# antgroup/ant-ray

Hardware: NVIDIA H100
Metric: resnet50_ddp_train_images_per_sec (higher is better)
Workload: dtype bf16

## Files before the change

ant-ray_b200/_native.py:

```python
import ctypes
import os
from ctypes import (POINTER, Structure, byref, c_char_p, c_float, c_int, c_int32, c_size_t, c_uint8,
                    c_uint32, c_uint64, c_void_p)

_LIB_NAME = "libb200coll.so"
_lib = None


class B200CollError(RuntimeError):

    def __init__(self, status, message):
        super().__init__(message)
        self.status = status

    def __reduce__(self):
        return (B200CollError, (self.status, self.args[0] if self.args else ""))


OK, EINVAL, ECUDA, ESTATE, EUNSUPPORTED, ETIMEOUT, EABORTED, EMISMATCH, ENOMEM = 0, -1, -2, -3, -4, -5, -6, -7, -8
INT8, UINT8, INT32, UINT32, INT64, UINT64, FLOAT16, FLOAT32, FLOAT64, BFLOAT16 = range(10)
SUM, PROD, MAX, MIN, AVG = range(5)
ALGO_AUTO, ALGO_ONESHOT, ALGO_TWOSHOT, ALGO_NVLS, ALGO_NVLS_PIPE, ALGO_LL, ALGO_NVLS_LANES, ALGO_NVLS_STREAMS = range(8)
SHARE_VMM_FD, SHARE_LEGACY_IPC = 0, 1
ACT_RELU6, ACT_SILU, ACT_HARDSWISH = 1, 2, 3
MAX_RANKS = 8


class Config(Structure):
    _fields_ = [("struct_size", c_uint32), ("share_mode", c_int32), ("staging_bytes", c_uint64),
                ("symmetric_bytes", c_uint64), ("p2p_slot_bytes", c_uint64), ("p2p_slots", c_uint32),
                ("max_blocks", c_uint32), ("oneshot_max_bytes", c_uint64), ("nvls_min_bytes", c_uint64),
                ("nvls_pipe_min_bytes", c_uint64), ("timeout_ms", c_uint64), ("granule_bytes", c_uint64),
                ("ll_max_bytes", c_uint64), ("bcast_rounds_min_bytes", c_uint64), ("nvls_blocks", c_uint32),
                ("nvls_lanes", c_uint32), ("lane_granule_bytes", c_uint64), ("nvls_lanes_min_bytes", c_uint64),
                ("nvls_unroll", c_uint32), ("rounds_order", c_uint32), ("nvls_streams_min_bytes", c_uint64),
                ("nvls_streams_piece_bytes", c_uint64)]


class Props(Structure):
    _fields_ = [("device", c_int32), ("sm_count", c_int32), ("cc_major", c_int32), ("cc_minor", c_int32),
                ("vmm_supported", c_int32), ("posix_fd_supported", c_int32), ("multicast_supported", c_int32),
                ("reserved", c_int32), ("total_mem", c_uint64)]


class Export(Structure):
    _fields_ = [("share_mode", c_int32), ("fd", c_int32), ("arena_bytes", c_uint64), ("layout_hash", c_uint64),
                ("pid", c_int32), ("device_uuid_lo", c_int32), ("ipc", c_uint8 * 64)]


SYMBOLS = {
    "b200c_version": (c_int, []),
    "b200c_last_error": (c_char_p, []),
    "b200c_status_string": (c_char_p, [c_int]),
    "b200c_dtype_size": (c_size_t, [c_int]),
    "b200c_device_props": (c_int, [c_int, POINTER(Props)]),
    "b200c_default_config": (None, [POINTER(Config)]),
    "b200c_comm_create": (c_int, [c_int, c_int, c_int, POINTER(Config), POINTER(c_void_p)]),
    "b200c_comm_export": (c_int, [c_void_p, POINTER(Export)]),
    "b200c_comm_import": (c_int, [c_void_p, c_int, POINTER(Export)]),
    "b200c_comm_mc_create": (c_int, [c_void_p, POINTER(c_int)]),
    "b200c_comm_mc_import": (c_int, [c_void_p, c_int]),
    "b200c_comm_mc_add_device": (c_int, [c_void_p]),
    "b200c_comm_mc_bind": (c_int, [c_void_p]),
    "b200c_comm_mc_disable": (c_int, [c_void_p]),
    "b200c_comm_ready": (c_int, [c_void_p]),
    "b200c_comm_abort": (c_int, [c_void_p]),
    "b200c_comm_destroy": (c_int, [c_void_p]),
    "b200c_comm_check": (c_int, [c_void_p]),
    "b200c_comm_rank": (c_int, [c_void_p]),
    "b200c_comm_world": (c_int, [c_void_p]),
    "b200c_comm_has_multicast": (c_int, [c_void_p]),
    "b200c_comm_seq": (c_uint64, [c_void_p]),
    "b200c_comm_symmetric_base": (c_void_p, [c_void_p]),
    "b200c_comm_symmetric_bytes": (c_uint64, [c_void_p]),
    "b200c_pool_bind": (c_int, [c_void_p]),
    "b200c_pool_malloc": (c_void_p, [c_size_t, c_int, c_void_p]),
    "b200c_pool_free": (None, [c_void_p, c_size_t, c_int, c_void_p]),
    "b200c_allreduce": (c_int, [c_void_p, c_void_p, c_void_p, c_size_t, c_int, c_int, c_int, c_void_p]),
    "b200c_allreduce_scaled": (c_int, [c_void_p, c_void_p, c_void_p, c_size_t, c_int, c_int, c_float, c_int, c_void_p]),
    "b200c_reduce": (c_int, [c_void_p, c_void_p, c_void_p, c_size_t, c_int, c_int, c_int, c_void_p]),
    "b200c_broadcast": (c_int, [c_void_p, c_void_p, c_size_t, c_int, c_int, c_void_p]),
    "b200c_allgather": (c_int, [c_void_p, c_void_p, POINTER(c_void_p), c_size_t, c_int, c_void_p]),
    "b200c_reducescatter": (c_int, [c_void_p, POINTER(c_void_p), c_void_p, c_size_t, c_int, c_int, c_void_p]),
    "b200c_reducescatter_scaled": (c_int, [c_void_p, POINTER(c_void_p), c_void_p, c_size_t, c_int, c_int, c_float, c_void_p]),
    "b200c_send": (c_int, [c_void_p, c_void_p, c_size_t, c_int, c_void_p]),
    "b200c_recv": (c_int, [c_void_p, c_void_p, c_size_t, c_int, c_void_p]),
    "b200c_send_multi": (c_int, [c_void_p, c_void_p, c_size_t, POINTER(c_int), c_int, c_void_p]),
    "b200c_recv_multi": (c_int, [c_void_p, c_void_p, c_size_t, c_int, c_void_p]),
    "b200c_barrier": (c_int, [c_void_p, c_void_p]),
    "b200c_debug_fill_flags": (c_int, [c_void_p, c_uint32]),
    "b200c_bn_scratch_bytes": (c_size_t, [c_int]),
    "b200c_bn_forward": (c_int, [c_void_p] * 10 + [c_int, c_int, c_float, c_float, c_void_p, c_void_p]),
    "b200c_bn_forward_mask": (c_int, [c_void_p] * 11 + [c_int, c_int, c_float, c_float, c_void_p, c_void_p]),
    "b200c_bn_backward": (c_int, [c_void_p] * 10 + [c_int, c_int, c_void_p, c_void_p]),
    "b200c_bn_backward_mask": (c_int, [c_void_p] * 11 + [c_int, c_int, c_void_p, c_void_p]),
    "b200c_bn_dual_scratch_bytes": (c_size_t, [c_int]),
    "b200c_bn_forward_dual": (c_int, [c_void_p] * 11 + [c_float, c_float] + [c_void_p] * 7 + [c_float, c_float, c_int, c_int, c_void_p, c_void_p]),
    "b200c_bn_backward_dual": (c_int, [c_void_p] * 18 + [c_int, c_int, c_void_p, c_void_p]),
    "b200c_bn_forward_pool": (c_int, [c_void_p] * 10 + [c_int] * 4 + [c_float, c_float, c_void_p, c_void_p]),
    "b200c_bn_backward_pool": (c_int, [c_void_p] * 10 + [c_int] * 4 + [c_void_p, c_void_p]),
    "b200c_bn_infer": (c_int, [c_void_p] * 7 + [c_int, c_float, c_int, c_int, c_void_p]),
    "b200c_bn_infer_dual": (c_int, [c_void_p] * 7 + [c_float] + [c_void_p] * 4 + [c_float, c_int, c_int, c_int, c_void_p]),
    "b200c_bn_infer_pool": (c_int, [c_void_p] * 6 + [c_int, c_float] + [c_int] * 4 + [c_void_p]),
    "b200c_bn_forward_act": (c_int, [c_void_p] * 9 + [c_int, c_int, c_int, c_float, c_float, c_void_p, c_void_p]),
    "b200c_bn_backward_act": (c_int, [c_void_p] * 10 + [c_int, c_int, c_int, c_void_p, c_void_p]),
    "b200c_bn_infer_act": (c_int, [c_void_p] * 6 + [c_int, c_float, c_int, c_int, c_int, c_void_p]),
    "b200c_bn_forward_res": (c_int, [c_void_p] * 3 + [c_int] + [c_void_p] * 8 + [c_int, c_int, c_float, c_float, c_void_p, c_void_p]),
    "b200c_bn_backward_res": (c_int, [c_void_p] * 2 + [c_int] + [c_void_p] * 8 + [c_int, c_int, c_void_p, c_void_p]),
    "b200c_bn_infer_res": (c_int, [c_void_p] * 7 + [c_int, c_float, c_int, c_int, c_void_p]),
    "b200c_bn_forward_cat": (c_int, [POINTER(c_void_p), POINTER(c_int), c_int] + [c_void_p] * 9 + [c_int, c_int, c_float, c_float, c_void_p,
                                                                                              c_void_p]),
    "b200c_bn_backward_cat": (c_int, [c_void_p] * 2 + [POINTER(c_void_p), POINTER(c_int), c_int] + [c_void_p] * 6 + [c_int, c_int, c_void_p,
                                                                                                                  c_void_p]),
    "b200c_bn_infer_cat": (c_int, [POINTER(c_void_p), POINTER(c_int), c_int] + [c_void_p] * 5 + [c_int, c_float, c_int, c_int, c_void_p]),
    "b200c_bn_forward_slice": (c_int, [c_void_p, c_void_p, c_int] + [c_void_p] * 8 + [c_int, c_int, c_float, c_float, c_void_p, c_void_p]),
    "b200c_bn_backward_slice": (c_int, [c_void_p, c_int] + [c_void_p] * 8 + [c_int, c_int, c_void_p, c_void_p]),
    "b200c_bn_infer_slice": (c_int, [c_void_p, c_void_p, c_int] + [c_void_p] * 4 + [c_int, c_float, c_int, c_int, c_void_p]),
    "b200c_bn_shuffle_mask_bytes": (c_size_t, [c_int, c_int]),
    "b200c_bn_forward_shuffle": (c_int, [c_void_p, c_int] + [c_void_p] * 9 + [c_float, c_float] + [c_void_p] * 9
                                 + [c_float, c_float, c_void_p, c_int, c_int, c_int, c_void_p, c_void_p]),
    "b200c_bn_backward_shuffle": (c_int, [c_void_p] * 17 + [c_int, c_int, c_void_p, c_void_p]),
    "b200c_bn_infer_shuffle": (c_int, [c_void_p, c_int] + [c_void_p] * 5 + [c_float] + [c_void_p] * 5
                               + [c_float, c_void_p, c_int, c_int, c_int, c_int, c_void_p]),
    "b200c_se_scratch_bytes": (c_size_t, [c_int, c_int, c_int]),
    "b200c_se_pool": (c_int, [c_void_p] * 2 + [c_int] * 3 + [c_void_p, c_size_t, c_void_p]),
    "b200c_se_scale": (c_int, [c_void_p] * 3 + [c_int] * 3 + [c_void_p]),
    "b200c_se_backward_reduce": (c_int, [c_void_p] * 3 + [c_int] * 3 + [c_void_p, c_size_t, c_void_p]),
    "b200c_se_backward_elemt": (c_int, [c_void_p] * 4 + [c_int] * 3 + [c_void_p]),
    "b200c_bn_sync_scratch_bytes": (c_size_t, [c_int, c_int]),
    "b200c_bn_sync_forward": (c_int, [c_void_p] * 5 + [c_int] + [c_void_p] * 8 + [c_int, c_int, c_float, c_float, c_void_p, c_void_p]),
    "b200c_bn_sync_backward": (c_int, [c_void_p] * 5 + [c_int] + [c_void_p] * 9 + [c_int, c_int, c_void_p, c_void_p]),
    "b200c_launch_count": (c_uint64, []),
}


def library_path():
    override = os.environ.get("B200COLL_LIBRARY")
    if override:
        return override
    return os.path.join(os.path.dirname(os.path.abspath(__file__)), _LIB_NAME)


def load():
    global _lib
    if _lib is not None:
        return _lib
    path = library_path()
    if not os.path.exists(path):
        raise ImportError(
            f"{path} not found: build it with `python -c 'import __graft_entry__ as g; g.build()'` "
            "(nvcc, sm_90a).  ant_ray_b200 has no CPU or NCCL fallback.")
    lib = ctypes.CDLL(path, mode=ctypes.RTLD_LOCAL)
    for name, (restype, argtypes) in SYMBOLS.items():
        fn = getattr(lib, name)
        fn.restype = restype
        fn.argtypes = argtypes
    if lib.b200c_version() < 200:
        raise ImportError("libb200coll.so is older than this Python package")
    _lib = lib
    return lib


def last_error():
    msg = load().b200c_last_error()
    return msg.decode(errors="replace") if msg else ""


def check(status):
    if status != OK:
        raise B200CollError(status, f"b200coll: {last_error()} (status {status})")


def default_config():
    cfg = Config()
    load().b200c_default_config(byref(cfg))
    return cfg


def device_props(device):
    p = Props()
    check(load().b200c_device_props(device, byref(p)))
    return p


def launch_count():
    return int(load().b200c_launch_count())
```

ant-ray_b200/csrc/b200coll.cu:

```cuda
#include <cuda.h>
#include <cuda_runtime.h>
#include <stdarg.h>
#include <stdio.h>
#include <stdlib.h>
#include <string.h>
#include <unistd.h>

#include <atomic>
#include <initializer_list>
#include <mutex>

#include "byte_kernels.cuh"
#include "launch_typed.cuh"
#include "norm_launch.h"
#include "se_launch.h"

using namespace b200c;

static thread_local char g_err[512] = "";
static int fail(int code, const char* fmt, ...) {
  va_list ap;
  va_start(ap, fmt);
  vsnprintf(g_err, sizeof g_err, fmt, ap);
  va_end(ap);
// ... 934 lines not shown
      c->tma_ctas_per_sm = nb;
    }
    size_t cap = (size_t)c->sm_count * c->tma_ctas_per_sm;
    int tgrid = (int)(ntiles < cap ? ntiles : cap);
    with_scaled_types(dtype, wire, [&](auto ti, auto tw) {
      k_local_scale_tma<typename decltype(ti)::type, typename decltype(tw)::type><<<tgrid, kTmaThreads, kTmaSmemBytes, s>>>(a);
    });
    int rc = launch_check(c, "local_scale_tma");
    if (rc) return rc;
    if (tma_elems == count) return B200C_OK;
    a.in = static_cast<const char*>(send) + tma_elems * esz;
    a.out = static_cast<char*>(recv) + tma_elems * esz;
    a.n = count - tma_elems;
  }
  int grid = local_scale_grid<float, bf16_t>(c, a.n * esz);
  if (dtype == B200C_FLOAT64) k_local_scale<double, double><<<grid, kThreads, 0, s>>>(a);
  else if (!with_scaled_types(dtype, wire, [&](auto ti, auto tw) {
             k_local_scale<typename decltype(ti)::type, typename decltype(tw)::type><<<grid, kThreads, 0, s>>>(a);
           }))
    return copy_if_distinct(send, recv, count * esz, s);
  return launch_check(c, "local_scale");
}

static int choose_algo(b200c_comm* c, int algo, size_t total_bytes, size_t bytes_left, bool ll_ok, bool nvls_ok, bool in_sym,
                       bool* pipe, bool* lanes) {
  const int W = c->world;
  int al = algo;
  if (al == B200C_ALGO_NVLS_PIPE) { al = B200C_ALGO_NVLS; *pipe = true; }
  if (al == B200C_ALGO_NVLS_LANES) { al = B200C_ALGO_NVLS; *lanes = true; }
  if (al == B200C_ALGO_AUTO) {
    if (ll_ok && total_bytes <= c->cfg.ll_max_bytes) al = B200C_ALGO_LL;
    else if (bytes_left <= c->cfg.oneshot_max_bytes) al = B200C_ALGO_ONESHOT;
    else if (nvls_ok && W > 2 && bytes_left >= c->cfg.nvls_min_bytes && (W >= 6 || in_sym)) al = B200C_ALGO_NVLS;
    else al = B200C_ALGO_TWOSHOT;
  }
  return al;
}

static void plan_ll(b200c_comm* c, CollArgs& a, size_t left, size_t esz, size_t vec, int& grid) {
  size_t n = left;
  a.chunk = round_up(n, vec);
  a.tile = vec;
  a.ll_seq = c->ll_seq + 1;
  size_t nvec = (n * esz + 15) / 16;
  size_t nb = (nvec + kLLThreads - 1) / kLLThreads;
  grid = (int)(nb < 1 ? 1 : (nb > c->cfg.max_blocks ? c->cfg.max_blocks : nb));
  a.n = n;
}
static void plan_oneshot(b200c_comm* c, CollArgs& a, size_t left, size_t wsz, size_t vec, int& grid) {
  const int W = c->world;
  size_t cap = c->cfg.staging_bytes / W / wsz / vec * vec;
  size_t n = left < cap ? left : cap;
  a.chunk = round_up(n, vec);
  plan_tiles(n, wsz, vec, c->cfg.max_blocks, kMinTileBytes, c->cfg.granule_bytes, &a.tile, &grid);
  a.n = n;
}
static void plan_twoshot(b200c_comm* c, CollArgs& a, size_t left, size_t wsz, size_t vec, int& grid) {
  const int W = c->world;
  size_t cap_chunk = c->cfg.staging_bytes / W / wsz / vec * vec;
  size_t cap = cap_chunk * W;
  size_t n = left < cap ? left : cap;
  a.chunk = round_up((n + W - 1) / W, vec);
  plan_tiles(a.chunk, wsz, vec, c->cfg.max_blocks, kMinTileBytes, c->cfg.granule_bytes, &a.tile, &grid);
  a.n = n;
}
static int plan_nvls(b200c_comm* c, CollArgs& a, size_t left, size_t wsz, size_t vec, bool sym, int algo, bool& pipe, bool& lanes,
                     int& grid, uint32_t& rounds) {
  const int W = c->world;
  const uint32_t nvls_sym_cap = c->cfg.nvls_blocks && c->cfg.nvls_blocks < c->cfg.max_blocks ? c->cfg.nvls_blocks : c->cfg.max_blocks;
  size_t cap = sym ? ((size_t)256 << 20) / wsz : c->cfg.staging_bytes / wsz / vec * vec;
  size_t n = left < cap ? left : cap;
  a.chunk = round_up((n + W - 1) / W, vec);
  a.symmetric = sym ? 1 : 0;
  a.sym_off = sym ? (size_t)((const char*)a.in - c->arena[c->rank]) : 0;
  if (!sym && algo == B200C_ALGO_AUTO && c->cfg.nvls_lanes_min_bytes && left * wsz >= c->cfg.nvls_lanes_min_bytes) lanes = true;
  if (!sym && !lanes && algo == B200C_ALGO_AUTO && c->cfg.nvls_pipe_min_bytes && n * wsz >= c->cfg.nvls_pipe_min_bytes) pipe = true;
  if (sym) pipe = lanes = false;
  if (lanes) {
    n = left;
    a.chunk = round_up((n + W - 1) / W, vec);
    uint32_t L = c->cfg.nvls_lanes;
    uint32_t Kc = c->cfg.max_blocks / L - 1;
    if (Kc > 7) Kc = 7;
    if (Kc < 1) Kc = 1;
    size_t tb = c->cfg.lane_granule_bytes, chunk_bytes = a.chunk * wsz;
    size_t want = chunk_bytes / ((size_t)L * 4) / 8192 * 8192;
    if (want < 8192) want = 8192;
    if (tb > want) tb = want;
    size_t ring = (size_t)L * kLaneSlots * W * tb;
    while (ring > c->cfg.staging_bytes && tb > 8192) { tb -= 8192; ring = (size_t)L * kLaneSlots * W * tb; }
    while (ring > c->cfg.staging_bytes && L > 1) { L--; ring = (size_t)L * kLaneSlots * W * tb; }
    if (ring > c->cfg.staging_bytes) return fail(B200C_EINVAL, "staging_bytes too small for the lane kernel's ring (%zu bytes)", ring);
    a.tile = tb / wsz;
    a.lane_copy = (int)Kc;
    size_t ngran = (a.chunk + a.tile - 1) / a.tile;
    uint32_t used = (uint32_t)(ngran < L ? ngran : L);
    grid = (int)(used * (1 + Kc));
    rounds = (uint32_t)((ngran + used - 1) / used);
    a.pipe_base = c->pipe_base;
  } else if (pipe) {
    plan_rounds(a.chunk, wsz, vec, c->cfg.max_blocks, c->cfg.granule_bytes, &a.tile, &grid, &rounds);
    a.pipe_base = c->pipe_base;
  } else {
    plan_tiles(a.chunk, wsz, vec, sym ? nvls_sym_cap : c->cfg.max_blocks, kMinTileBytes, c->cfg.granule_bytes, &a.tile, &grid);
  }
  a.n = n;
  return B200C_OK;
}

static int allreduce_impl(b200c_comm* c, const void* send, void* recv, size_t count, int dtype, int wire, int op, float scale,
                          int has_scale, int algo, cudaStream_t s) {
  int rc = check_ready(c);
  if (rc) return rc;
  size_t esz = b200c_dtype_size(dtype), wsz = b200c_dtype_size(wire);
  if (!esz || !wsz) return fail(B200C_EINVAL, "bad dtype %d / wire %d", dtype, wire);
  if (op < 0 || op >= B200C_NUM_OPS) return fail(B200C_EINVAL, "bad reduce op %d", op);
  if (count && (!send || !recv)) return fail(B200C_EINVAL, "null buffer");
  if (wire != dtype) {
    if (!(dtype == B200C_FLOAT32 && (wire == B200C_BFLOAT16 || wire == B200C_FLOAT16))) return fail(B200C_EUNSUPPORTED, "wire dtype %d for buffer dtype %d", wire, dtype);
    if (op != B200C_SUM && op != B200C_AVG) return fail(B200C_EUNSUPPORTED, "compressed wire supports SUM/AVG only");
  }
  if (algo < B200C_ALGO_AUTO || algo > B200C_ALGO_NVLS_STREAMS) return fail(B200C_EINVAL, "bad algo %d", algo);
  if (op == B200C_AVG) { has_scale = 1; scale = 1.f / (float)c->world; }
  if (count == 0) return B200C_OK;
  DeviceGuard g(c->device);
  const int W = c->world;
  const size_t vec = 16 / wsz;
  if (W == 1) return allreduce_local(c, send, recv, count, dtype, wire, scale, has_scale, s);

  const bool nvls_ok = c->mc_arena && (op == B200C_SUM || op == B200C_AVG) &&
                       (wire == B200C_FLOAT32 || wire == B200C_BFLOAT16 || wire == B200C_FLOAT16);
  if ((algo == B200C_ALGO_NVLS || algo == B200C_ALGO_NVLS_PIPE || algo == B200C_ALGO_NVLS_LANES || algo == B200C_ALGO_NVLS_STREAMS) && !nvls_ok) return fail(B200C_EUNSUPPORTED, "NVLS needs a bound multicast object, SUM/AVG and f32/bf16/f16");
  const bool ll_ok = wire == dtype && c->ll_words && count * esz <= c->ll_words * 4;
  if (algo == B200C_ALGO_LL && !ll_ok) return fail(B200C_EUNSUPPORTED, "LL needs wire == dtype and at most %zu bytes (ll_max_bytes)", c->ll_words * 4);
  const char* in = static_cast<const char*>(send);
  char* out = static_cast<char*>(recv);
  bool in_sym = false;
  if (wire == dtype && send == recv && c->sym_bytes && (((uintptr_t)send) & 15) == 0 && (count * esz) % 16 == 0) {
    const char* base = c->arena[c->rank] + c->off_sym;
    in_sym = in >= base && in + count * esz <= base + c->sym_bytes;
  }
  if (!in_sym && (algo == B200C_ALGO_NVLS_STREAMS ||
                  (algo == B200C_ALGO_AUTO && nvls_ok && W >= 6 && c->cfg.nvls_streams_min_bytes && count * wsz >= c->cfg.nvls_streams_min_bytes)))
    return allreduce_streams(c, send, recv, count, dtype, wire, op, scale, has_scale, s);
  return run_pieces(c, count, count, "allreduce", [&](CollArgs& a, size_t done, uint32_t& rounds) -> int {
    const size_t left = count - done;
    bool pipe = false, lanes = false;
    const int al = choose_algo(c, algo, count * esz, left * wsz, ll_ok, nvls_ok, in_sym, &pipe, &lanes);
    a.in = in + done * esz; a.out = out + done * esz;
    a.has_scale = has_scale; a.scale = scale;
    const bool sym = al == B200C_ALGO_NVLS && in_sym;
    int grid = 0;
    if (al == B200C_ALGO_LL) plan_ll(c, a, left, esz, vec, grid);
    else if (al == B200C_ALGO_ONESHOT) plan_oneshot(c, a, left, wsz, vec, grid);
    else if (al == B200C_ALGO_TWOSHOT) plan_twoshot(c, a, left, wsz, vec, grid);
    else {
      int rc = plan_nvls(c, a, left, wsz, vec, sym, algo, pipe, lanes, grid, rounds);
      if (rc) return rc;
    }
    a.sig = make_sig(OPC_ALLREDUCE, dtype * 16 + wire, op, a.n, sym ? (int)((a.sym_off >> 4) & 0x3fffffff) : -1, al * 8 + (sym ? 1 : 0) + (pipe ? 2 : 0) + (lanes ? 4 : 0));
    if (al == B200C_ALGO_NVLS) launch_nvls(dtype, wire, a, grid, s, pipe, lanes);
    else if (wire != dtype) {
      if (wire == B200C_BFLOAT16) launch_mixed<float, bf16_t>(al, a, grid, s);
      else launch_mixed<float, f16_t>(al, a, grid, s);
    } else {
      int kind = al == B200C_ALGO_LL ? KIND_LL : (al == B200C_ALGO_ONESHOT ? KIND_ONESHOT : KIND_TWOSHOT);
      return launch_same_type(dtype, kind, op, a, grid, s);
    }
    return B200C_OK;
  });
}

extern "C" int b200c_allreduce(b200c_comm_t* c, const void* send, void* recv, size_t count, int dtype, int op, int algo,
                               b200c_stream_t stream) {
  return allreduce_impl(c, send, recv, count, dtype, dtype, op, 1.f, 0, algo, (cudaStream_t)stream);
}

extern "C" int b200c_allreduce_scaled(b200c_comm_t* c, const void* send, void* recv, size_t count, int dtype, int wire_dtype,
                                      float scale, int algo, b200c_stream_t stream) {
  if (dtype != B200C_FLOAT32 && dtype != B200C_BFLOAT16 && dtype != B200C_FLOAT16)
    return fail(B200C_EUNSUPPORTED, "scaled allreduce supports f32/bf16/f16 buffers, got %d", dtype);
  return allreduce_impl(c, send, recv, count, dtype, wire_dtype, B200C_SUM, scale, 1, algo, (cudaStream_t)stream);
}

extern "C" int b200c_reduce(b200c_comm_t* c, const void* send, void* recv, size_t count, int dtype, int op, int root,
                            b200c_stream_t stream) {
  int rc = check_ready(c);
  if (rc) return rc;
  size_t esz = b200c_dtype_size(dtype);
  if (!esz) return fail(B200C_EINVAL, "bad dtype %d", dtype);
  if (op < 0 || op >= B200C_NUM_OPS) return fail(B200C_EINVAL, "bad reduce op %d", op);
  if (root < 0 || root >= c->world) return fail(B200C_EINVAL, "bad root %d", root);
  if (count == 0) return B200C_OK;
  if (!send || (c->rank == root && !recv)) return fail(B200C_EINVAL, "null buffer");
  cudaStream_t s = (cudaStream_t)stream;
  DeviceGuard g(c->device);
  if (c->world == 1) return copy_if_distinct(send, recv, count * esz, s);
  const size_t vec = 16 / esz;
  size_t cap = c->cfg.staging_bytes / c->world / esz / vec * vec;
  return run_pieces(c, count, cap, "reduce", [&](CollArgs& a, size_t done, uint32_t&) {
    a.in = static_cast<const char*>(send) + done * esz;
    a.out = recv ? static_cast<char*>(recv) + done * esz : nullptr;
    a.chunk = round_up(a.n, vec); a.root = root;
    if (op == B200C_AVG) { a.has_scale = 1; a.scale = 1.f / c->world; }
    int grid;
    plan_tiles(a.n, esz, vec, c->cfg.max_blocks, kMinTileBytes, c->cfg.granule_bytes, &a.tile, &grid);
    a.sig = make_sig(OPC_REDUCE, dtype, op, a.n, root, 0);
    return launch_same_type(dtype, KIND_REDUCE, op, a, grid, s);
  });
}

extern "C" int b200c_reducescatter(b200c_comm_t* c, const void* const* send_ptrs, void* recv, size_t count, int dtype, int op,
                                   b200c_stream_t stream) {
  int rc = check_ready(c);
  if (rc) return rc;
  size_t esz = b200c_dtype_size(dtype);
  if (!esz) return fail(B200C_EINVAL, "bad dtype %d", dtype);
  if (op < 0 || op >= B200C_NUM_OPS) return fail(B200C_EINVAL, "bad reduce op %d", op);
  if (count == 0) return B200C_OK;
  if (!send_ptrs || !recv) return fail(B200C_EINVAL, "null buffer");
  for (int j = 0; j < c->world; j++) if (!send_ptrs[j]) return fail(B200C_EINVAL, "send_ptrs[%d] is null", j);
  cudaStream_t s = (cudaStream_t)stream;
  DeviceGuard g(c->device);
  if (c->world == 1) return copy_if_distinct(send_ptrs[0], recv, count * esz, s);
  const size_t vec = 16 / esz;
  size_t cap = c->cfg.staging_bytes / c->world / esz / vec * vec;
  return run_pieces(c, count, cap, "reducescatter", [&](CollArgs& a, size_t done, uint32_t&) {
    for (int j = 0; j < c->world; j++) a.in_ptrs[j] = static_cast<const char*>(send_ptrs[j]) + done * esz;
    a.out = static_cast<char*>(recv) + done * esz;
    a.chunk = round_up(a.n, vec);
    if (op == B200C_AVG) { a.has_scale = 1; a.scale = 1.f / c->world; }
    int grid;
    plan_tiles(a.n, esz, vec, c->cfg.max_blocks, kMinTileBytes, c->cfg.granule_bytes, &a.tile, &grid);
    a.sig = make_sig(OPC_REDUCESCATTER, dtype, op, a.n, -1, 0);
    return launch_same_type(dtype, KIND_REDUCESCATTER, op, a, grid, s);
  });
}

extern "C" int b200c_reducescatter_scaled(b200c_comm_t* c, const void* const* send_ptrs, void* recv, size_t count, int dtype,
                                          int wire_dtype, float scale, b200c_stream_t stream) {
  int rc = check_ready(c);
  if (rc) return rc;
  if (dtype != B200C_FLOAT32 && dtype != B200C_BFLOAT16 && dtype != B200C_FLOAT16)
    return fail(B200C_EUNSUPPORTED, "scaled reducescatter supports f32/bf16/f16 buffers, got %d", dtype);
  const size_t esz = b200c_dtype_size(dtype), wsz = b200c_dtype_size(wire_dtype);
  if (!wsz) return fail(B200C_EINVAL, "bad wire dtype %d", wire_dtype);
  if (wire_dtype != dtype && !(dtype == B200C_FLOAT32 && (wire_dtype == B200C_BFLOAT16 || wire_dtype == B200C_FLOAT16)))
    return fail(B200C_EUNSUPPORTED, "wire dtype %d for buffer dtype %d", wire_dtype, dtype);
  if (count == 0) return B200C_OK;
  if (!send_ptrs || !recv) return fail(B200C_EINVAL, "null buffer");
  for (int j = 0; j < c->world; j++) if (!send_ptrs[j]) return fail(B200C_EINVAL, "send_ptrs[%d] is null", j);
  cudaStream_t s = (cudaStream_t)stream;
  if (c->world == 1) return allreduce_impl(c, send_ptrs[0], recv, count, dtype, wire_dtype, B200C_SUM, scale, 1, B200C_ALGO_AUTO, s);
  DeviceGuard g(c->device);
  const size_t vec = 16 / wsz;
  size_t cap = c->cfg.staging_bytes / c->world / wsz / vec * vec;
  return run_pieces(c, count, cap, "reducescatter_scaled", [&](CollArgs& a, size_t done, uint32_t&) {
    for (int j = 0; j < c->world; j++) a.in_ptrs[j] = static_cast<const char*>(send_ptrs[j]) + done * esz;
    a.out = static_cast<char*>(recv) + done * esz;
    a.chunk = round_up(a.n, vec);
    a.has_scale = 1; a.scale = scale;
    int grid;
    plan_tiles(a.n, wsz, vec, c->cfg.max_blocks, kMinTileBytes, c->cfg.granule_bytes, &a.tile, &grid);
    a.sig = make_sig(OPC_REDUCESCATTER, dtype, B200C_SUM, a.n, -1, 16 + wire_dtype);
    launch_rs_scaled(dtype, wire_dtype, a, grid, s);
    return B200C_OK;
  });
}

extern "C" int b200c_allgather(b200c_comm_t* c, const void* send, void* const* recv_ptrs, size_t count, int dtype,
                               b200c_stream_t stream) {
  int rc = check_ready(c);
  if (rc) return rc;
  size_t esz = b200c_dtype_size(dtype);
  if (!esz) return fail(B200C_EINVAL, "bad dtype %d", dtype);
  if (count == 0) return B200C_OK;
  if (!send || !recv_ptrs) return fail(B200C_EINVAL, "null buffer");
  for (int j = 0; j < c->world; j++) if (!recv_ptrs[j]) return fail(B200C_EINVAL, "recv_ptrs[%d] is null", j);
  cudaStream_t s = (cudaStream_t)stream;
  DeviceGuard g(c->device);
  size_t bytes = count * esz;
  if (c->world == 1) return copy_if_distinct(send, recv_ptrs[0], bytes, s);
  size_t cap = c->cfg.staging_bytes / c->world / 16 * 16;
  return run_pieces(c, bytes, cap, "allgather", [&](CollArgs& a, size_t done, uint32_t&) {
    a.in = static_cast<const char*>(send) + done;
    for (int j = 0; j < c->world; j++) a.out_ptrs[j] = static_cast<char*>(recv_ptrs[j]) + done;
    a.chunk = round_up(a.n, 16);
    int grid;
    plan_tiles(a.n, 1, 16, c->cfg.max_blocks, kMinTileBytes, c->cfg.granule_bytes, &a.tile, &grid);
    a.sig = make_sig(OPC_ALLGATHER, dtype, 0, a.n, -1, 0);
    k_allgather<<<grid, kThreads, 0, s>>>(a);
    return B200C_OK;
  });
}

extern "C" size_t b200c_bn_scratch_bytes(int channels) {
  return channels < 1 || channels > bn::kMaxChannels ? 0 : bn::scratch_bytes(channels);
}

extern "C" size_t b200c_bn_sync_scratch_bytes(int channels, int world) {
  return channels < 1 || channels > bn::kMaxChannels || world < 1 || world > kMaxRanks ? 0 : bn::sync_scratch_bytes(channels, world);
}

static const char* bn_site(bool sync) { return sync ? "sync batch norm" : "batch norm"; }

static int check_bn(const char* site, int min_m, int m, int c, const void* scratch, int relu, const void* mask, const void* residual,
                    const void* dy2) {
  if (m < min_m || c < 1 || c > bn::kMaxChannels || (int64_t)m * c > INT32_MAX)
    return fail(B200C_EINVAL, "%s: bad shape m=%d c=%d", site, m, c);
  if (!scratch) return fail(B200C_EINVAL, "%s: null scratch", site);
  if (!relu && (mask || residual || dy2)) return fail(B200C_EINVAL, "%s: a site without ReLU takes no mask, identity or dy2", site);
  if (mask && c % 8) return fail(B200C_EINVAL, "%s mask: channels=%d is not a multiple of 8", site, c);
  return B200C_OK;
}

static int bn_forward(b200c_comm_t* comm, bool sync, const void* x, const void* identity, void* y, void* mask, int relu,
                      const float* weight, const float* bias, float* running_mean, float* running_var, int64_t* num_batches_tracked,
                      float* save_mean, float* save_invstd, float* norm_fct, int m, int channels, float momentum, float eps,
                      void* scratch, b200c_stream_t stream) {
  int rc = check_bn(bn_site(sync), sync ? 0 : 1, m, channels, scratch, relu, mask, identity, nullptr);
  if (rc) return rc;
  if ((m && (!x || !y)) || !weight || !bias || !running_mean || !running_var || !save_mean || !save_invstd || (sync && !norm_fct))
    return fail(B200C_EINVAL, "%s forward: null buffer", bn_site(sync));
  const bn::FwdArgs a{x, identity, y, mask, relu != 0, weight, bias, running_mean, running_var,
                      reinterpret_cast<long long*>(num_batches_tracked), save_mean, save_invstd, m, channels, momentum, eps, scratch};
  cudaStream_t s = (cudaStream_t)stream;
  if (!sync) {
    RT(bn::forward(a, s));
    g_launches.fetch_add(2);
    return B200C_OK;
  }
  rc = check_ready(comm);
  if (rc) return rc;
  DeviceGuard g(comm->device);
  const int rows = m != 0;
  RT(bn::sync_stats(a, s));
  g_launches.fetch_add(rows);
  const bn::SyncRows r = bn::sync_rows(scratch, channels);
  void* gathered[kMaxRanks];
  for (int j = 0; j < comm->world; j++) gathered[j] = r.gathered + j * r.row_floats;
  rc = b200c_allgather(comm, r.local, gathered, (size_t)2 * channels + 1, B200C_FLOAT32, stream);
  if (rc) return rc;
  RT(bn::sync_apply(a, comm->world, norm_fct, s));
  g_launches.fetch_add(1 + rows);
  return B200C_OK;
}

static int bn_backward(b200c_comm_t* comm, bool sync, const void* dy, const void* dy2, const void* y, const void* mask, int relu,
                       const void* x, void* dy_masked, void* dx, const float* weight, const float* save_mean, const float* save_invstd,
                       const float* norm_fct, float* grad_weight, float* grad_bias, int m, int channels, void* scratch,
                       b200c_stream_t stream) {
  int rc = check_bn(bn_site(sync), sync ? 0 : 1, m, channels, scratch, relu, mask, dy_masked, dy2);
  if (rc) return rc;
  if ((m && (!dy || !x || !dx || (relu && !y && !mask))) || !weight || !save_mean || !save_invstd || (sync && !norm_fct) ||
      !grad_weight || !grad_bias)
    return fail(B200C_EINVAL, "%s backward: null buffer", bn_site(sync));
  const bn::BwdArgs a{dy, dy2, y, mask, x, dy_masked, dx, relu != 0, weight, save_mean, save_invstd, norm_fct, grad_weight, grad_bias,
                      m, channels, scratch};
  cudaStream_t s = (cudaStream_t)stream;
  if (!sync) {
    RT(bn::backward(a, s));
    g_launches.fetch_add(2);
    return B200C_OK;
  }
  rc = check_ready(comm);
  if (rc) return rc;
  DeviceGuard g(comm->device);
  const int rows = m != 0;
  RT(bn::sync_bwd_reduce(a, s));
  g_launches.fetch_add(rows);
  float* sums = bn::sync_rows(scratch, channels).sums;
  rc = b200c_allreduce(comm, sums, sums, (size_t)2 * channels, B200C_FLOAT32, B200C_SUM, B200C_ALGO_AUTO, stream);
  if (rc) return rc;
  RT(bn::sync_bwd_elemt(a, s));
  g_launches.fetch_add(rows);
  return B200C_OK;
}

extern "C" int b200c_bn_forward(const void* x, const void* identity, void* y, const float* weight, const float* bias,
                                float* running_mean, float* running_var, int64_t* num_batches_tracked, float* save_mean,
                                float* save_invstd, int m, int channels, float momentum, float eps, void* scratch,
                                b200c_stream_t stream) {
  return bn_forward(nullptr, false, x, identity, y, nullptr, 1, weight, bias, running_mean, running_var, num_batches_tracked, save_mean,
                    save_invstd, nullptr, m, channels, momentum, eps, scratch, stream);
}

extern "C" int b200c_bn_forward_mask(const void* x, const void* identity, void* y, uint8_t* mask, const float* weight,
                                     const float* bias, float* running_mean, float* running_var, int64_t* num_batches_tracked,
                                     float* save_mean, float* save_invstd, int m, int channels, float momentum, float eps,
                                     void* scratch, b200c_stream_t stream) {
  if (!mask) return fail(B200C_EINVAL, "batch norm mask: null mask");
  return bn_forward(nullptr, false, x, identity, y, mask, 1, weight, bias, running_mean, running_var, num_batches_tracked, save_mean,
                    save_invstd, nullptr, m, channels, momentum, eps, scratch, stream);
}

extern "C" int b200c_bn_sync_forward(b200c_comm_t* comm, const void* x, const void* identity, void* y, uint8_t* mask, int relu,
                                     const float* weight, const float* bias, float* running_mean, float* running_var,
                                     int64_t* num_batches_tracked, float* save_mean, float* save_invstd, float* norm_fct, int m,
                                     int channels, float momentum, float eps, void* scratch, b200c_stream_t stream) {
  return bn_forward(comm, true, x, identity, y, mask, relu, weight, bias, running_mean, running_var, num_batches_tracked, save_mean,
                    save_invstd, norm_fct, m, channels, momentum, eps, scratch, stream);
}

extern "C" int b200c_bn_backward(const void* dy, const void* y, const void* x, void* dy_masked, void* dx, const float* weight,
                                 const float* save_mean, const float* save_invstd, float* grad_weight, float* grad_bias, int m,
                                 int channels, void* scratch, b200c_stream_t stream) {
  return bn_backward(nullptr, false, dy, nullptr, y, nullptr, 1, x, dy_masked, dx, weight, save_mean, save_invstd, nullptr, grad_weight,
                     grad_bias, m, channels, scratch, stream);
}

extern "C" int b200c_bn_backward_mask(const void* dy, const void* dy2, const uint8_t* mask, const void* x, void* dy_masked,
                                      void* dx, const float* weight, const float* save_mean, const float* save_invstd,
                                      float* grad_weight, float* grad_bias, int m, int channels, void* scratch,
                                      b200c_stream_t stream) {
  if (!mask) return fail(B200C_EINVAL, "batch norm mask: null mask");
  return bn_backward(nullptr, false, dy, dy2, nullptr, mask, 1, x, dy_masked, dx, weight, save_mean, save_invstd, nullptr, grad_weight,
                     grad_bias, m, channels, scratch, stream);
}

extern "C" int b200c_bn_sync_backward(b200c_comm_t* comm, const void* dy, const void* dy2, const void* y, const uint8_t* mask, int relu,
                                      const void* x, void* dy_masked, void* dx, const float* weight, const float* save_mean,
                                      const float* save_invstd, const float* norm_fct, float* grad_weight, float* grad_bias, int m,
                                      int channels, void* scratch, b200c_stream_t stream) {
  return bn_backward(comm, true, dy, dy2, y, mask, relu, x, dy_masked, dx, weight, save_mean, save_invstd, norm_fct, grad_weight,
                     grad_bias, m, channels, scratch, stream);
}

extern "C" size_t b200c_bn_dual_scratch_bytes(int channels) {
  return channels < 1 || channels > bn::kMaxChannels / 2 ? 0 : bn::dual_scratch_bytes(channels);
}

static int check_dual(int channels) {
  if (channels > bn::kMaxChannels / 2) return fail(B200C_EINVAL, "batch norm dual: channels=%d above %d", channels, bn::kMaxChannels / 2);
  return B200C_OK;
}

extern "C" int b200c_bn_forward_dual(const void* x, const void* x_ds, void* y, uint8_t* mask, const float* weight, const float* bias,
                                     float* running_mean, float* running_var, int64_t* num_batches_tracked, float* save_mean,
                                     float* save_invstd, float momentum, float eps, const float* weight_ds, const float* bias_ds,
                                     float* running_mean_ds, float* running_var_ds, int64_t* num_batches_tracked_ds,
                                     float* save_mean_ds, float* save_invstd_ds, float momentum_ds, float eps_ds, int m, int channels,
                                     void* scratch, b200c_stream_t stream) {
  int rc = check_bn("batch norm dual", 1, m, channels, scratch, 1, mask, x_ds, nullptr);
  if (!rc) rc = check_dual(channels);
  if (rc) return rc;
  if (!x || !x_ds || !y || !weight || !bias || !running_mean || !running_var || !save_mean || !save_invstd || !weight_ds ||
      !bias_ds || !running_mean_ds || !running_var_ds || !save_mean_ds || !save_invstd_ds)
    return fail(B200C_EINVAL, "batch norm dual forward: null buffer");
  const bn::FwdArgs a{x, nullptr, y, mask, true, weight, bias, running_mean, running_var,
                      reinterpret_cast<long long*>(num_batches_tracked), save_mean, save_invstd, m, channels, momentum, eps, scratch};
  const bn::FwdArgs b{x_ds, nullptr, nullptr, nullptr, false, weight_ds, bias_ds, running_mean_ds, running_var_ds,
                      reinterpret_cast<long long*>(num_batches_tracked_ds), save_mean_ds, save_invstd_ds, m, channels, momentum_ds,
                      eps_ds, scratch};
  RT(bn::forward_dual(a, b, (cudaStream_t)stream));
  g_launches.fetch_add(2);
  return B200C_OK;
}

extern "C" int b200c_bn_backward_dual(const void* dy, const void* dy2, const void* y, const uint8_t* mask, const void* x,
                                      const void* x_ds, void* dx, void* dx_ds, const float* weight, const float* save_mean,
                                      const float* save_invstd, float* grad_weight, float* grad_bias, const float* weight_ds,
                                      const float* save_mean_ds, const float* save_invstd_ds, float* grad_weight_ds,
                                      float* grad_bias_ds, int m, int channels, void* scratch, b200c_stream_t stream) {
  int rc = check_bn("batch norm dual", 1, m, channels, scratch, 1, mask, nullptr, dy2);
  if (!rc) rc = check_dual(channels);
  if (rc) return rc;
  if (!dy || (!y && !mask) || !x || !x_ds || !dx || !dx_ds || !weight || !save_mean || !save_invstd || !grad_weight || !grad_bias ||
      !weight_ds || !save_mean_ds || !save_invstd_ds || !grad_weight_ds || !grad_bias_ds)
    return fail(B200C_EINVAL, "batch norm dual backward: null buffer");
  const bn::BwdArgs a{dy, dy2, mask ? nullptr : y, mask, x, nullptr, dx, true, weight, save_mean, save_invstd, nullptr, grad_weight,
                      grad_bias, m, channels, scratch};
  const bn::BwdArgs b{nullptr, nullptr, nullptr, nullptr, x_ds, nullptr, dx_ds, false, weight_ds, save_mean_ds, save_invstd_ds, nullptr,
                      grad_weight_ds, grad_bias_ds, m, channels, scratch};
  RT(bn::backward_dual(a, b, (cudaStream_t)stream));
  g_launches.fetch_add(2);
  return B200C_OK;
}

static int check_pool(const char* dir, int n, int h, int w, int channels, int* m) {
  if (n < 1 || h < 1 || w < 1 || (int64_t)n * h * w > INT32_MAX)
    return fail(B200C_EINVAL, "batch norm pool %s: bad shape n=%d h=%d w=%d c=%d", dir, n, h, w, channels);
  *m = n * h * w;
  return B200C_OK;
}

extern "C" int b200c_bn_forward_pool(const void* x, void* y, uint8_t* argmax, const float* weight, const float* bias,
                                     float* running_mean, float* running_var, int64_t* num_batches_tracked, float* save_mean,
                                     float* save_invstd, int n, int h, int w, int channels, float momentum, float eps, void* scratch,
                                     b200c_stream_t stream) {
  int m = 0;
  int rc = check_pool("forward", n, h, w, channels, &m);
  if (!rc) rc = check_bn("batch norm pool", 1, m, channels, scratch, 1, nullptr, nullptr, nullptr);
  if (rc) return rc;
  if (!x || !y || !argmax || !weight || !bias || !running_mean || !running_var || !save_mean || !save_invstd)
    return fail(B200C_EINVAL, "batch norm pool forward: null buffer");
  bn::FwdArgs a{x, nullptr, y, nullptr, true, weight, bias, running_mean, running_var,
                reinterpret_cast<long long*>(num_batches_tracked), save_mean, save_invstd, m, channels, momentum, eps, scratch};
  a.argmax = argmax;
  a.pool_h = h;
  a.pool_w = w;
  RT(bn::forward(a, (cudaStream_t)stream));
  g_launches.fetch_add(2);
  return B200C_OK;
}

extern "C" int b200c_bn_backward_pool(const void* dy, const uint8_t* argmax, const void* x, void* g, void* dx, const float* weight,
                                      const float* save_mean, const float* save_invstd, float* grad_weight, float* grad_bias, int n,
                                      int h, int w, int channels, void* scratch, b200c_stream_t stream) {
  int m = 0;
  int rc = check_pool("backward", n, h, w, channels, &m);
  if (!rc) rc = check_bn("batch norm pool", 1, m, channels, scratch, 1, nullptr, nullptr, nullptr);
  if (rc) return rc;
  if (!dy || !argmax || !x || !g || !dx || !weight || !save_mean || !save_invstd || !grad_weight || !grad_bias)
    return fail(B200C_EINVAL, "batch norm pool backward: null buffer");
  bn::BwdArgs a{dy, nullptr, nullptr, nullptr, x, g, dx, true, weight, save_mean, save_invstd, nullptr, grad_weight, grad_bias,
                m, channels, scratch};
  a.argmax = argmax;
  a.pool_h = h;
  a.pool_w = w;
  RT(bn::backward(a, (cudaStream_t)stream));
  g_launches.fetch_add(2);
  return B200C_OK;
}

static int check_infer(const char* site, int param_bf16, int m, int c) {
  if (m < 1 || c < 1 || (int64_t)m * c > INT32_MAX) return fail(B200C_EINVAL, "%s: bad shape m=%d c=%d", site, m, c);
  if (param_bf16 != 0 && param_bf16 != 1) return fail(B200C_EINVAL, "%s: param_bf16=%d is neither 0 nor 1", site, param_bf16);
  return B200C_OK;
}

static int run_infer(const bn::InferArgs& a, b200c_stream_t stream) {
  RT(bn::infer(a, (cudaStream_t)stream));
  g_launches.fetch_add(1);
  return B200C_OK;
}

extern "C" int b200c_bn_infer(const void* x, const void* identity, void* y, const void* weight, const void* bias,
                              const void* running_mean, const void* running_var, int param_bf16, float eps, int m, int channels,
                              b200c_stream_t stream) {
  int rc = check_infer("batch norm infer", param_bf16, m, channels);
  if (rc) return rc;
  if (!x || !y || !weight || !bias || !running_mean || !running_var) return fail(B200C_EINVAL, "batch norm infer: null buffer");
  return run_infer({x, identity, y, {weight, bias, running_mean, running_var, eps}, {}, false, param_bf16 != 0, m, channels, 0, 0},
                   stream);
}

extern "C" int b200c_bn_infer_dual(const void* x, const void* x_ds, void* y, const void* weight, const void* bias,
                                   const void* running_mean, const void* running_var, float eps, const void* weight_ds,
                                   const void* bias_ds, const void* running_mean_ds, const void* running_var_ds, float eps_ds,
                                   int param_bf16, int m, int channels, b200c_stream_t stream) {
  int rc = check_infer("batch norm infer dual", param_bf16, m, channels);
  if (rc) return rc;
  if (!x || !x_ds || !y || !weight || !bias || !running_mean || !running_var || !weight_ds || !bias_ds || !running_mean_ds ||
      !running_var_ds)
    return fail(B200C_EINVAL, "batch norm infer dual: null buffer");
  return run_infer({x, x_ds, y, {weight, bias, running_mean, running_var, eps}, {weight_ds, bias_ds, running_mean_ds, running_var_ds, eps_ds},
                    true, param_bf16 != 0, m, channels, 0, 0},
                   stream);
}

extern "C" int b200c_bn_infer_pool(const void* x, void* y, const void* weight, const void* bias, const void* running_mean,
                                   const void* running_var, int param_bf16, float eps, int n, int h, int w, int channels,
                                   b200c_stream_t stream) {
  int m = 0;
  int rc = check_pool("infer", n, h, w, channels, &m);
  if (!rc) rc = check_infer("batch norm infer pool", param_bf16, m, channels);
  if (rc) return rc;
  if (!x || !y || !weight || !bias || !running_mean || !running_var) return fail(B200C_EINVAL, "batch norm infer pool: null buffer");
  return run_infer({x, nullptr, y, {weight, bias, running_mean, running_var, eps}, {}, false, param_bf16 != 0, m, channels, h, w}, stream);
}

static int check_act(const char* site, int act, int c) {
  if (!bn::act_ok(act)) return fail(B200C_EINVAL, "%s: unknown act=%d", site, act);
  if (c > bn::kMaxChannels) return fail(B200C_EINVAL, "%s: channels=%d above %d", site, c, bn::kMaxChannels);
  return B200C_OK;
}

extern "C" int b200c_bn_forward_act(const void* x, void* y, const float* weight, const float* bias, float* running_mean,
                                    float* running_var, int64_t* num_batches_tracked, float* save_mean, float* save_invstd, int act,
                                    int m, int channels, float momentum, float eps, void* scratch, b200c_stream_t stream) {
  int rc = check_bn("batch norm act", 1, m, channels, scratch, 1, nullptr, nullptr, nullptr);
  if (!rc) rc = check_act("batch norm act", act, channels);
  if (rc) return rc;
  if (!x || !y || !weight || !bias || !running_mean || !running_var || !save_mean || !save_invstd)
    return fail(B200C_EINVAL, "batch norm act forward: null buffer");
  const bn::FwdArgs a{x, nullptr, y, nullptr, false, weight, bias, running_mean, running_var,
                      reinterpret_cast<long long*>(num_batches_tracked), save_mean, save_invstd, m, channels, momentum, eps, scratch};
  RT(bn::forward_act(a, act, (cudaStream_t)stream));
  g_launches.fetch_add(2);
  return B200C_OK;
}

extern "C" int b200c_bn_backward_act(const void* dy, const void* x, void* g, void* dx, const float* weight, const float* bias,
                                     const float* save_mean, const float* save_invstd, float* grad_weight, float* grad_bias, int act,
                                     int m, int channels, void* scratch, b200c_stream_t stream) {
  int rc = check_bn("batch norm act", 1, m, channels, scratch, 1, nullptr, nullptr, nullptr);
  if (!rc) rc = check_act("batch norm act", act, channels);
  if (rc) return rc;
  if (!dy || !x || !g || !dx || !weight || !bias || !save_mean || !save_invstd || !grad_weight || !grad_bias)
    return fail(B200C_EINVAL, "batch norm act backward: null buffer");
  const bn::BwdArgs a{dy, nullptr, nullptr, nullptr, x, g, dx, false, weight, save_mean, save_invstd, nullptr, grad_weight, grad_bias,
                      m, channels, scratch};
  RT(bn::backward_act(a, bias, act, (cudaStream_t)stream));
  g_launches.fetch_add(2);
  return B200C_OK;
}
// ... 461 lines not shown
```

ant-ray_b200/csrc/inst_norm.cu:

```cuda
#include <algorithm>
#include <initializer_list>
#include <type_traits>

#include "norm_act.cuh"
#include "norm_cat.cuh"
#include "norm_infer.cuh"
#include "norm_kernels.cuh"
#include "norm_launch.h"
#include "norm_res.cuh"
#include "norm_shuffle.cuh"
#include "norm_slice.cuh"

namespace b200c {
namespace bn {

static int ceil_div(int a, int b) { return (a + b - 1) / b; }

static int last_pow2(unsigned n) {
  n |= (n >> 1);
  n |= (n >> 2);
  n |= (n >> 4);
  n |= (n >> 8);
  n |= (n >> 16);
  return std::max<int>(1, n - (n >> 1));
}

static void reduce_config(int reduction, int stride, dim3* block, dim3* grid) {
  int block_x = std::min(last_pow2(stride), kTileW);
  int block_y = std::min(last_pow2(ceil_div(reduction, kElemsPerThread)), kMaxBlock / block_x);
  if (block_x * block_y != kMaxBlock) block_x = std::min(last_pow2(stride), kMaxBlock / block_y);
  int grid_y = std::min(ceil_div(reduction, block_y * kElemsPerThread), kMaxHBlock);
  *block = dim3(block_x, block_y, 1);
  *grid = dim3(ceil_div(stride, block_x), grid_y < 8 ? 1 : grid_y, 1);
}

static_assert(kEwVec % kStatsVec == 0, "vec_ok covers the statistics kernel's vector width");
static bool vec_ok(int stride, const void* const* ptrs, int n) {
  if (stride % kEwVec) return false;
  for (int i = 0; i < n; i++)
    if (reinterpret_cast<uintptr_t>(ptrs[i]) % 16) return false;
  return true;
}

constexpr size_t kBlockSmem = 48 * 1024;
constexpr size_t kStatsStaticSmem = 3 * kMaxBlock * 4 + 16;
constexpr size_t kBwdStaticSmem = 2 * kMaxBlock * 4 + 16;

static size_t stats_ring_bytes(dim3 block) {
  return (size_t)kStatsStages * kParallelLoads * block.x * block.y * sizeof(BVec<kStatsVec>);
}
static_assert(kStatsStaticSmem + (size_t)kStatsStages * kParallelLoads * (kMaxBlock / kStatsVec) * sizeof(BVec<kStatsVec>) <= kBlockSmem,
              "the statistics ring fits every block");

static_assert(kBwdStaticSmem + (size_t)kBwdStagesWide * 5 * kParallelLoads * (kMaxBlock / kBwdVec) * sizeof(BVec<kBwdVec>) <= kBlockSmem &&
                  kBwdStaticSmem + (size_t)kBwdStages * 2 * kParallelLoads * (kMaxBlock / kBwdVec) * sizeof(BVec<kBwdVec>) <= kBlockSmem,
              "the backward ring fits every block: 2 stages of up to 5 operands, 3 of 2");
struct BwdReduceLaunch {
  dim3 block, grid;
  int vec;
  size_t smem;
};
static BwdReduceLaunch bwd_reduce_launch(int m, int c, GradSrc src, bool dy2, bool dual, const void* const* ptrs, int n) {
  BwdReduceLaunch l;
  reduce_config(m, c, &l.block, &l.grid);
  l.vec = 1;
  l.smem = 0;
  if (src == kGradPool || !vec_ok(c, ptrs, n)) return l;
  const int ops = bwd_ring_operands(src == kGradY, dy2, dual);
  const size_t ring = (size_t)bwd_ring_stages(ops) * ops * kParallelLoads * (l.block.x / kBwdVec) * l.block.y * sizeof(BVec<kBwdVec>);
  l.block.x /= kBwdVec;
  l.vec = kBwdVec;
  l.smem = ring;
  return l;
}

static void ew_config(int reduction, int stride, int vec, dim3* block, dim3* grid) {
  const int groups = stride / vec;
  const int bx = std::min(groups, kEwThreads);
  const int by = kEwThreads / bx;
  const int gx = ceil_div(groups, bx);
  const int gy = std::max(1, std::min(ceil_div(reduction, by), 4096 / gx));
  *block = dim3(bx, by, 1);
  *grid = dim3(gx, gy, 1);
}

constexpr int kSemaphores = kMaxChannels / kTileW;
constexpr size_t kSemaphoreBytes = (size_t)kSemaphores * 4;

size_t scratch_bytes(int stride) {
  return kSemaphoreBytes + (size_t)3 * stride * kMaxHBlock * 4 + (size_t)2 * stride * 4;
}

struct Scratch {
  int* semaphores;
  float* staging;
  float* sums;
};
static Scratch carve(void* scratch, int stride) {
  char* p = static_cast<char*>(scratch);
  Scratch s;
  s.semaphores = reinterpret_cast<int*>(p);
  s.staging = reinterpret_cast<float*>(p + kSemaphoreBytes);
  s.sums = s.staging + (size_t)3 * stride * kMaxHBlock;
  return s;
}

template <int... Cs, typename F>
static auto with_const(int key, F&& f) {
  std::common_type_t<decltype(f(std::integral_constant<int, Cs>{}))...> kernel = nullptr;
  ((key == Cs ? void(kernel = f(std::integral_constant<int, Cs>{})) : void()), ...);
  return kernel;
}

using StatsKernel = void (*)(const bf16*, StatsOut, volatile float*, int*, int, int);
using SyncStatsKernel = void (*)(const bf16*, float*, float, volatile float*, int*, int, int);
using StatsDualKernel = void (*)(const bf16*, const bf16*, StatsOut, StatsOut, volatile float*, volatile float*, int*, int, int);
using TransformKernel = void (*)(const bf16*, const bf16*, bf16*, uint8_t*, const float*, const float*, const float*, const float*,
                                 const float*, const float*, const float*, const float*, int, int);
using PoolFwdKernel = void (*)(const bf16*, bf16*, uint8_t*, const float*, const float*, const float*, const float*, PoolDims, int, int);
using BwdReduceKernel = void (*)(const bf16*, const bf16*, const bf16*, const bf16*, const uint8_t*, bf16*, const float*, const float*,
                                 float*, float*, float*, float*, volatile float*, int*, PoolDims, const bf16*, const float*, const float*,
                                 float*, float*, float*, int, int, int);
using BwdElemtKernel = void (*)(const bf16*, const bf16*, const bf16*, const uint8_t*, const bf16*, bf16*, const float*, const float*,
                                const float*, const float*, const float*, const float*, float, const bf16*, bf16*, const float*,
                                const float*, const float*, const float*, int, int);

static StatsKernel stats_kernel(int vec) {
  return with_const<1, kStatsVec>(vec, [](auto v) -> StatsKernel { return k_bn_stats<decltype(v)::value>; });
}
static StatsDualKernel stats_dual_kernel(int vec) {
  return with_const<1, kStatsVec>(vec, [](auto v) -> StatsDualKernel { return k_bn_stats_dual<decltype(v)::value>; });
}
static SyncStatsKernel sync_stats_kernel(int vec) {
  return with_const<1, kStatsVec>(vec, [](auto v) -> SyncStatsKernel { return k_bn_sync_stats<decltype(v)::value>; });
}
static TransformKernel transform_kernel(int vec, int tail) {
  return with_const<1, kEwVec>(vec, [&](auto v) {
    return with_const<kTailNone, kTailRelu, kTailAddRelu, kTailBnAddRelu>(
        tail, [](auto t) -> TransformKernel { return k_bn_transform<decltype(v)::value, (Tail) decltype(t)::value>; });
  });
}
static PoolFwdKernel pool_fwd_kernel(int vec) {
  return with_const<1, kEwVec>(vec, [](auto v) -> PoolFwdKernel { return k_bn_pool_fwd<decltype(v)::value>; });
}
static BwdReduceKernel bwd_reduce_kernel(int src, bool dual) {
  if (dual)
    return with_const<kGradY, kGradBits>(src, [](auto g) -> BwdReduceKernel { return k_bn_bwd_reduce<(GradSrc) decltype(g)::value, true>; });
  return with_const<kGradY, kGradBits, kGradDy, kGradPool>(
      src, [](auto g) -> BwdReduceKernel { return k_bn_bwd_reduce<(GradSrc) decltype(g)::value, false>; });
}
static BwdElemtKernel bwd_elemt_kernel(int vec, int src, bool fct_ptr, bool dual) {
  return with_const<1, kEwVec>(vec, [&](auto v) {
    if (dual)
      return with_const<kGradY, kGradBits>(src, [](auto g) -> BwdElemtKernel {
        return k_bn_bwd_elemt<decltype(v)::value, (GradSrc) decltype(g)::value, false, true>;
      });
    return with_const<kGradMasked, kGradY, kGradBits, kGradDy>(src, [&](auto g) {
      auto kernel = [](auto p) -> BwdElemtKernel {
        return k_bn_bwd_elemt<decltype(v)::value, (GradSrc) decltype(g)::value, decltype(p)::value != 0, false>;
      };
      if constexpr (decltype(g)::value == kGradDy) return with_const<true>(fct_ptr, kernel);
      else return with_const<false, true>(fct_ptr, kernel);
    });
  });
}

template <typename P>
using InferTransformKernel = void (*)(const bf16*, const bf16*, bf16*, const P*, const P*, const P*, const P*, float, const P*, const P*,
                                      const P*, const P*, float, int, int);
template <typename P>
using InferPoolKernel = void (*)(const bf16*, bf16*, const P*, const P*, const P*, const P*, float, PoolDims, int, int);

template <typename P>
static InferTransformKernel<P> infer_transform_kernel(int vec, int tail) {
  return with_const<1, kEwVec>(vec, [&](auto v) {
    return with_const<kTailRelu, kTailAddRelu, kTailBnAddRelu>(tail, [](auto t) -> InferTransformKernel<P> {
      return bn_infer::k_infer_transform<decltype(v)::value, (Tail) decltype(t)::value, P>;
    });
  });
}
template <typename P>
static InferPoolKernel<P> infer_pool_kernel(int vec) {
  return with_const<1, kEwVec>(vec, [](auto v) -> InferPoolKernel<P> { return bn_infer::k_infer_pool<decltype(v)::value, P>; });
}

using bn_act::Act;
using ActTransformKernel = void (*)(const bf16*, bf16*, const float*, const float*, const float*, const float*, int, int);
using ActBwdReduceKernel = void (*)(const bf16*, const bf16*, const float*, const float*, const float*, const float*, float*, float*,
                                    float*, float*, volatile float*, int*, bf16*, int, int);
template <typename P>
using ActInferKernel = void (*)(const bf16*, bf16*, const P*, const P*, const P*, const P*, float, int, int);

template <typename F>
static auto with_act(int act, F&& f) {
  return with_const<bn_act::kActRelu6, bn_act::kActSilu, bn_act::kActHardswish>(act, f);
}
bool act_ok(int act) { return act == bn_act::kActRelu6 || act == bn_act::kActSilu || act == bn_act::kActHardswish; }

static ActTransformKernel act_transform_kernel(int vec, int act) {
  return with_const<1, kEwVec>(vec, [&](auto v) {
    return with_act(act, [](auto a) -> ActTransformKernel { return bn_act::k_act_transform<decltype(v)::value, (Act) decltype(a)::value>; });
  });
}
static ActBwdReduceKernel act_bwd_reduce_kernel(int act) {
  return with_act(act, [](auto a) -> ActBwdReduceKernel { return bn_act::k_act_bwd_reduce<(Act) decltype(a)::value>; });
}
template <typename P>
static ActInferKernel<P> act_infer_kernel(int vec, int act) {
  return with_const<1, kEwVec>(vec, [&](auto v) {
    return with_act(act, [](auto a) -> ActInferKernel<P> { return bn_act::k_act_infer<decltype(v)::value, (Act) decltype(a)::value, P>; });
  });
}

using bn_res::Res;
using ResTransformKernel = void (*)(const bf16*, const bf16*, const bf16*, bf16*, const float*, const float*, const float*, const float*,
                                    int, int, int);
using ResBwdReduceKernel = void (*)(const bf16*, const bf16*, const bf16*, const float*, const float*, float*, float*, float*, float*,
                                    volatile float*, int*, bf16*, int, int, int);
template <typename P>
using ResInferKernel = void (*)(const bf16*, const bf16*, bf16*, const P*, const P*, const P*, const P*, float, int, int);

static ResTransformKernel res_transform_kernel(int vec, bool drop) {
  return with_const<1, kEwVec>(vec, [&](auto v) -> ResTransformKernel {
    return drop ? bn_res::k_res_transform<decltype(v)::value, bn_res::kResDropAdd> : bn_res::k_res_transform<decltype(v)::value, bn_res::kResAdd>;
  });
}
static ResBwdReduceKernel res_bwd_reduce_kernel() { return bn_res::k_res_bwd_reduce; }
template <typename P>
static ResInferKernel<P> res_infer_kernel(int vec, bool add) {
  return with_const<1, kEwVec>(vec, [&](auto v) -> ResInferKernel<P> {
    return add ? bn_res::k_res_infer<decltype(v)::value, bn_res::kResAdd, P> : bn_res::k_res_infer<decltype(v)::value, bn_res::kResPlain, P>;
  });
}

cudaError_t load_kernels() {
  cudaFuncAttributes attr;
  cudaError_t e = cudaSuccess;
  auto load = [&](auto kernel) { if (kernel && e == cudaSuccess) e = cudaFuncGetAttributes(&attr, kernel); };
  load(&k_bn_sync_merge);
  load(res_bwd_reduce_kernel());
  load(&bn_cat::k_cat_stats);
  load(&bn_cat::k_cat_transform);
  load(&bn_cat::k_cat_bwd_reduce);
  load(&bn_cat::k_cat_bwd_elemt);
  load(&bn_cat::k_cat_infer<float>);
  load(&bn_cat::k_cat_infer<bf16>);
  load(&bn_slice::k_slice_transform);
  load(&bn_slice::k_slice_bwd_reduce);
  load(&bn_slice::k_slice_bwd_elemt);
  load(&bn_slice::k_slice_infer<float>);
  load(&bn_slice::k_slice_infer<bf16>);
  load(&bn_shuffle::k_shuffle_transform<false>);
  load(&bn_shuffle::k_shuffle_transform<true>);
  load(&bn_shuffle::k_shuffle_bwd_reduce<false>);
  load(&bn_shuffle::k_shuffle_bwd_reduce<true>);
  load(&bn_shuffle::k_shuffle_bwd_elemt<false>);
  load(&bn_shuffle::k_shuffle_bwd_elemt<true>);
  load(&bn_shuffle::k_shuffle_infer<false, float>);
  load(&bn_shuffle::k_shuffle_infer<true, float>);
  load(&bn_shuffle::k_shuffle_infer<false, bf16>);
  load(&bn_shuffle::k_shuffle_infer<true, bf16>);
  for (int src = 0; src < kGradSrcs; src++) {
    load(bwd_reduce_kernel(src, false));
    load(bwd_reduce_kernel(src, true));
  }
  for (int vec : {1, kStatsVec, kEwVec}) {
    load(stats_kernel(vec));
    load(stats_dual_kernel(vec));
    load(sync_stats_kernel(vec));
    load(pool_fwd_kernel(vec));
    for (int tail = 0; tail < kTails; tail++) load(transform_kernel(vec, tail));
    for (int src = 0; src < kGradSrcs; src++)
      for (bool fct_ptr : {false, true})
        for (bool dual : {false, true}) load(bwd_elemt_kernel(vec, src, fct_ptr, dual));
    load(infer_pool_kernel<float>(vec));
    load(infer_pool_kernel<bf16>(vec));
    for (int tail = 0; tail < kTails; tail++) {
      load(infer_transform_kernel<float>(vec, tail));
      load(infer_transform_kernel<bf16>(vec, tail));
    }
    for (int act : {bn_act::kActRelu6, bn_act::kActSilu, bn_act::kActHardswish}) {
      if (vec == 1) load(act_bwd_reduce_kernel(act));
      load(act_transform_kernel(vec, act));
      load(act_infer_kernel<float>(vec, act));
      load(act_infer_kernel<bf16>(vec, act));
    }
    for (bool b : {false, true}) {
      load(res_transform_kernel(vec, b));
      load(res_infer_kernel<float>(vec, b));
      load(res_infer_kernel<bf16>(vec, b));
    }
  }
  return e;
}

constexpr cudaError_t kNoKernel = cudaErrorInvalidDeviceFunction;

static cudaError_t launch_stats(const FwdArgs& a, float* sync_row, cudaStream_t st) {
  Scratch s = carve(a.scratch, a.c);
  dim3 block, grid;
  reduce_config(a.m, a.c, &block, &grid);
  const int vec = vec_ok(a.c, &a.x, 1) ? kStatsVec : 1;
  block.x /= vec;
  const size_t smem = vec == kStatsVec ? stats_ring_bytes(block) : 0;
  const bf16* x = static_cast<const bf16*>(a.x);
  if (sync_row) {
    const SyncStatsKernel k = sync_stats_kernel(vec);
    if (!k) return kNoKernel;
    k<<<grid, block, smem, st>>>(x, sync_row, a.eps, s.staging, s.semaphores, a.m, a.c);
  } else {
    const StatsKernel k = stats_kernel(vec);
    if (!k) return kNoKernel;
    StatsOut o{a.save_mean, a.save_invstd, a.running_mean, a.running_var, a.num_batches_tracked, a.momentum,
               (float)((double)a.m / (double)(a.m - 1)), a.eps};
    k<<<grid, block, smem, st>>>(x, o, s.staging, s.semaphores, a.m, a.c);
  }
  return cudaGetLastError();
}

static cudaError_t launch_transform(const FwdArgs& a, cudaStream_t st) {
  const void* ptrs[3] = {a.x, a.y, a.identity ? a.identity : a.x};
  const int vec = vec_ok(a.c, ptrs, 3) ? kEwVec : 1;
  dim3 block, grid;
  ew_config(a.m, a.c, vec, &block, &grid);
  const TransformKernel k = transform_kernel(vec, !a.relu ? kTailNone : a.identity ? kTailAddRelu : kTailRelu);
  if (!k) return kNoKernel;
  k<<<grid, block, 0, st>>>(static_cast<const bf16*>(a.x), static_cast<const bf16*>(a.identity), static_cast<bf16*>(a.y),
                            static_cast<uint8_t*>(a.mask), a.save_mean, a.save_invstd, a.weight, a.bias, nullptr, nullptr, nullptr,
                            nullptr, a.m, a.c);
  return cudaGetLastError();
}

static PoolDims pool_dims(int h, int w) { return PoolDims{h, w, (h - 1) / 2 + 1, (w - 1) / 2 + 1}; }

static cudaError_t launch_pool_fwd(const FwdArgs& a, cudaStream_t st) {
  const PoolDims d = pool_dims(a.pool_h, a.pool_w);
  const int pooled_rows = a.m / (a.pool_h * a.pool_w) * d.oh * d.ow;
  const void* ptrs[3] = {a.x, a.y, a.argmax};
  const int vec = vec_ok(a.c, ptrs, 3) ? kEwVec : 1;
  dim3 block, grid;
  ew_config(pooled_rows, a.c, vec, &block, &grid);
  const PoolFwdKernel k = pool_fwd_kernel(vec);
  if (!k) return kNoKernel;
  k<<<grid, block, 0, st>>>(static_cast<const bf16*>(a.x), static_cast<bf16*>(a.y), static_cast<uint8_t*>(a.argmax), a.save_mean,
                            a.save_invstd, a.weight, a.bias, d, pooled_rows, a.c);
  return cudaGetLastError();
}

cudaError_t forward(const FwdArgs& a, cudaStream_t st) {
  const cudaError_t e = launch_stats(a, nullptr, st);
  if (e != cudaSuccess) return e;
  return a.pool_h ? launch_pool_fwd(a, st) : launch_transform(a, st);
}

static GradSrc grad_src(const BwdArgs& a, bool reduced) {
  if (!a.relu) return kGradDy;
  if (reduced && a.dy_masked) return kGradMasked;
  if (a.pool_h) return kGradPool;
  return a.mask ? kGradBits : kGradY;
}

static cudaError_t launch_bwd_reduce(const BwdArgs& a, cudaStream_t st) {
  Scratch s = carve(a.scratch, a.c);
  const GradSrc src = grad_src(a, false);
  const void* ptrs[5] = {a.x, a.dy, a.dy2 ? a.dy2 : a.dy, src == kGradY ? a.y : a.dy, a.dy_masked ? a.dy_masked : a.dy};
  const BwdReduceLaunch l = bwd_reduce_launch(a.m, a.c, src, a.dy2 != nullptr, false, ptrs, 5);
  const BwdReduceKernel k = bwd_reduce_kernel(src, false);
  if (!k) return kNoKernel;
  const void* mask = src == kGradPool ? a.argmax : a.mask;
  k<<<l.grid, l.block, l.smem, st>>>(static_cast<const bf16*>(a.x), static_cast<const bf16*>(a.dy), static_cast<const bf16*>(a.dy2),
                            static_cast<const bf16*>(a.y), static_cast<const uint8_t*>(mask), static_cast<bf16*>(a.dy_masked),
                            a.save_mean, a.save_invstd, s.sums, s.sums + a.c, a.grad_weight, a.grad_bias, s.staging, s.semaphores,
                            pool_dims(a.pool_h, a.pool_w), nullptr, nullptr, nullptr, nullptr, nullptr, nullptr, a.m, a.c, l.vec);
  return cudaGetLastError();
}

static cudaError_t launch_bwd_elemt(const BwdArgs& a, cudaStream_t st) {
  Scratch s = carve(a.scratch, a.c);
  const GradSrc src = grad_src(a, true);
  const void* g = src == kGradMasked ? a.dy_masked : a.dy;
  const void* ptrs[5] = {a.x, a.dx, g, a.dy2 && src != kGradMasked ? a.dy2 : a.dy, a.y};
  const int vec = vec_ok(a.c, ptrs, src == kGradY ? 5 : 4) ? kEwVec : 1;
  dim3 block, grid;
  ew_config(a.m, a.c, vec, &block, &grid);
  const BwdElemtKernel k = bwd_elemt_kernel(vec, src, a.norm_fct != nullptr, false);
  if (!k) return kNoKernel;
  k<<<grid, block, 0, st>>>(static_cast<const bf16*>(g), static_cast<const bf16*>(a.dy2), static_cast<const bf16*>(a.y),
                            static_cast<const uint8_t*>(a.mask), static_cast<const bf16*>(a.x), static_cast<bf16*>(a.dx), a.save_mean,
                            a.save_invstd, a.weight, s.sums, s.sums + a.c, a.norm_fct, (float)(1.0 / a.m), nullptr, nullptr, nullptr,
                            nullptr, nullptr, nullptr, a.m, a.c);
  return cudaGetLastError();
}

cudaError_t backward(const BwdArgs& a, cudaStream_t st) {
  const cudaError_t e = launch_bwd_reduce(a, st);
  return e == cudaSuccess ? launch_bwd_elemt(a, st) : e;
}

static size_t dual_extra_offset(int c) { return (scratch_bytes(c) + 15) / 16 * 16; }
size_t dual_scratch_bytes(int c) { return dual_extra_offset(c) + (size_t)3 * c * kMaxHBlock * 4 + (size_t)c * 4; }
static float* dual_staging(void* scratch, int c) { return reinterpret_cast<float*>(static_cast<char*>(scratch) + dual_extra_offset(c)); }
static float* dual_sum_xmu2(void* scratch, int c) { return dual_staging(scratch, c) + (size_t)3 * c * kMaxHBlock; }

static cudaError_t launch_stats_dual(const FwdArgs& a, const FwdArgs& b, cudaStream_t st) {
  Scratch s = carve(a.scratch, a.c);
  dim3 block, grid;
  reduce_config(a.m, a.c, &block, &grid);
  const void* xs[2] = {a.x, b.x};
  const int svec = vec_ok(a.c, xs, 2) ? kStatsVec : 1;
  block.x /= svec;
  grid.z = 2;
  const size_t smem = svec == kStatsVec ? stats_ring_bytes(block) : 0;
  const StatsDualKernel ks = stats_dual_kernel(svec);
  if (!ks) return kNoKernel;
  StatsOut oa{a.save_mean, a.save_invstd, a.running_mean, a.running_var, a.num_batches_tracked, a.momentum,
              (float)((double)a.m / (double)(a.m - 1)), a.eps};
  StatsOut ob{b.save_mean, b.save_invstd, b.running_mean, b.running_var, b.num_batches_tracked, b.momentum,
              (float)((double)b.m / (double)(b.m - 1)), b.eps};
  ks<<<grid, block, smem, st>>>(static_cast<const bf16*>(a.x), static_cast<const bf16*>(b.x), oa, ob, s.staging,
                             dual_staging(a.scratch, a.c), s.semaphores, a.m, a.c);
  return cudaGetLastError();
}

cudaError_t forward_dual(const FwdArgs& a, const FwdArgs& b, cudaStream_t st) {
  const cudaError_t e = launch_stats_dual(a, b, st);
  if (e != cudaSuccess) return e;
  dim3 block, grid;
  const void* ptrs[3] = {a.x, a.y, b.x};
  const int vec = vec_ok(a.c, ptrs, 3) ? kEwVec : 1;
  ew_config(a.m, a.c, vec, &block, &grid);
  const TransformKernel kt = transform_kernel(vec, kTailBnAddRelu);
  if (!kt) return kNoKernel;
  kt<<<grid, block, 0, st>>>(static_cast<const bf16*>(a.x), static_cast<const bf16*>(b.x), static_cast<bf16*>(a.y),
                             static_cast<uint8_t*>(a.mask), a.save_mean, a.save_invstd, a.weight, a.bias, b.save_mean, b.save_invstd,
                             b.weight, b.bias, a.m, a.c);
  return cudaGetLastError();
}

cudaError_t backward_dual(const BwdArgs& a, const BwdArgs& b, cudaStream_t st) {
  Scratch s = carve(a.scratch, a.c);
  float* sum2 = dual_sum_xmu2(a.scratch, a.c);
  const GradSrc src = a.mask ? kGradBits : kGradY;
  const void* rptrs[5] = {a.x, a.dy, a.dy2 ? a.dy2 : a.dy, src == kGradY ? a.y : a.dy, b.x};
  const BwdReduceLaunch l = bwd_reduce_launch(a.m, a.c, src, a.dy2 != nullptr, true, rptrs, 5);
  const BwdReduceKernel kr = bwd_reduce_kernel(src, true);
  if (!kr) return kNoKernel;
  kr<<<l.grid, l.block, l.smem, st>>>(static_cast<const bf16*>(a.x), static_cast<const bf16*>(a.dy), static_cast<const bf16*>(a.dy2),
                             static_cast<const bf16*>(a.y), static_cast<const uint8_t*>(a.mask), nullptr, a.save_mean, a.save_invstd,
                             s.sums, s.sums + a.c, a.grad_weight, a.grad_bias, s.staging, s.semaphores, pool_dims(0, 0),
                             static_cast<const bf16*>(b.x), b.save_mean, b.save_invstd, sum2, b.grad_weight, b.grad_bias, a.m, a.c, l.vec);
  cudaError_t e = cudaGetLastError();
  if (e != cudaSuccess) return e;
  const void* ptrs[7] = {a.x, a.dx, a.dy, a.dy2 ? a.dy2 : a.dy, b.x, b.dx, a.y};
  const int vec = vec_ok(a.c, ptrs, src == kGradY ? 7 : 6) ? kEwVec : 1;
  dim3 block, grid;
  ew_config(a.m, a.c, vec, &block, &grid);
  const BwdElemtKernel ke = bwd_elemt_kernel(vec, src, false, true);
  if (!ke) return kNoKernel;
  ke<<<grid, block, 0, st>>>(static_cast<const bf16*>(a.dy), static_cast<const bf16*>(a.dy2), static_cast<const bf16*>(a.y),
                             static_cast<const uint8_t*>(a.mask), static_cast<const bf16*>(a.x), static_cast<bf16*>(a.dx), a.save_mean,
                             a.save_invstd, a.weight, s.sums, s.sums + a.c, nullptr, (float)(1.0 / a.m), static_cast<const bf16*>(b.x),
                             static_cast<bf16*>(b.dx), b.save_mean, b.save_invstd, b.weight, sum2, a.m, a.c);
  return cudaGetLastError();
}

template <typename P>
static cudaError_t launch_infer(const InferArgs& a, cudaStream_t st) {
  auto p = [](const void* q) { return static_cast<const P*>(q); };
  const bf16* x = static_cast<const bf16*>(a.x);
  bf16* y = static_cast<bf16*>(a.y);
  const InferParams& b = a.bn;
  dim3 block, grid;
  if (a.pool_h) {
    const PoolDims d = pool_dims(a.pool_h, a.pool_w);
    const int pooled_rows = a.m / (a.pool_h * a.pool_w) * d.oh * d.ow;
    const void* ptrs[2] = {a.x, a.y};
    const int vec = vec_ok(a.c, ptrs, 2) ? kEwVec : 1;
    ew_config(pooled_rows, a.c, vec, &block, &grid);
    const InferPoolKernel<P> k = infer_pool_kernel<P>(vec);
    if (!k) return kNoKernel;
    k<<<grid, block, 0, st>>>(x, y, p(b.running_mean), p(b.running_var), p(b.weight), p(b.bias), b.eps, d, pooled_rows, a.c);
    return cudaGetLastError();
  }
  const void* ptrs[3] = {a.x, a.y, a.identity ? a.identity : a.x};
  const int vec = vec_ok(a.c, ptrs, 3) ? kEwVec : 1;
  ew_config(a.m, a.c, vec, &block, &grid);
  const InferTransformKernel<P> k = infer_transform_kernel<P>(vec, a.dual ? kTailBnAddRelu : a.identity ? kTailAddRelu : kTailRelu);
  if (!k) return kNoKernel;
  const InferParams& ds = a.ds;
  k<<<grid, block, 0, st>>>(x, static_cast<const bf16*>(a.identity), y, p(b.running_mean), p(b.running_var), p(b.weight), p(b.bias), b.eps,
                            p(ds.running_mean), p(ds.running_var), p(ds.weight), p(ds.bias), ds.eps, a.m, a.c);
  return cudaGetLastError();
}

cudaError_t infer(const InferArgs& a, cudaStream_t st) { return a.param_bf16 ? launch_infer<bf16>(a, st) : launch_infer<float>(a, st); }

static cudaError_t launch_elemt_of(const BwdArgs& a, const bf16* g, cudaStream_t st) {
  Scratch s = carve(a.scratch, a.c);
  const void* ptrs[3] = {a.x, a.dx, g};
  const int vec = vec_ok(a.c, ptrs, 3) ? kEwVec : 1;
  dim3 block, grid;
  ew_config(a.m, a.c, vec, &block, &grid);
  const BwdElemtKernel ke = bwd_elemt_kernel(vec, kGradMasked, false, false);
  if (!ke) return kNoKernel;
  ke<<<grid, block, 0, st>>>(g, nullptr, nullptr, nullptr, static_cast<const bf16*>(a.x), static_cast<bf16*>(a.dx), a.save_mean,
                             a.save_invstd, a.weight, s.sums, s.sums + a.c, nullptr, (float)(1.0 / a.m), nullptr, nullptr, nullptr,
                             nullptr, nullptr, nullptr, a.m, a.c);
  return cudaGetLastError();
}

cudaError_t forward_act(const FwdArgs& a, int act, cudaStream_t st) {
  const cudaError_t e = launch_stats(a, nullptr, st);
  if (e != cudaSuccess) return e;
  const void* ptrs[2] = {a.x, a.y};
  const int vec = vec_ok(a.c, ptrs, 2) ? kEwVec : 1;
  dim3 block, grid;
  ew_config(a.m, a.c, vec, &block, &grid);
  const ActTransformKernel k = act_transform_kernel(vec, act);
  if (!k) return kNoKernel;
  k<<<grid, block, 0, st>>>(static_cast<const bf16*>(a.x), static_cast<bf16*>(a.y), a.save_mean, a.save_invstd, a.weight, a.bias, a.m, a.c);
  return cudaGetLastError();
}

cudaError_t backward_act(const BwdArgs& a, const float* bias, int act, cudaStream_t st) {
  Scratch s = carve(a.scratch, a.c);
  dim3 block, grid;
  reduce_config(a.m, a.c, &block, &grid);
  const ActBwdReduceKernel kr = act_bwd_reduce_kernel(act);
  if (!kr) return kNoKernel;
  const bf16* x = static_cast<const bf16*>(a.x);
  bf16* g = static_cast<bf16*>(a.dy_masked);
  kr<<<grid, block, 0, st>>>(x, static_cast<const bf16*>(a.dy), a.save_mean, a.save_invstd, a.weight, bias, s.sums, s.sums + a.c,
                             a.grad_weight, a.grad_bias, s.staging, s.semaphores, g, a.m, a.c);
  cudaError_t e = cudaGetLastError();
  if (e != cudaSuccess) return e;
  return launch_elemt_of(a, g, st);
}

template <typename P>
static cudaError_t launch_infer_act(const InferArgs& a, int act, cudaStream_t st) {
  const void* ptrs[2] = {a.x, a.y};
  const int vec = vec_ok(a.c, ptrs, 2) ? kEwVec : 1;
  dim3 block, grid;
  ew_config(a.m, a.c, vec, &block, &grid);
  const ActInferKernel<P> k = act_infer_kernel<P>(vec, act);
  if (!k) return kNoKernel;
  const InferParams& b = a.bn;
  k<<<grid, block, 0, st>>>(static_cast<const bf16*>(a.x), static_cast<bf16*>(a.y), static_cast<const P*>(b.running_mean),
                            static_cast<const P*>(b.running_var), static_cast<const P*>(b.weight), static_cast<const P*>(b.bias), b.eps,
                            a.m, a.c);
  return cudaGetLastError();
}

cudaError_t infer_act(const InferArgs& a, int act, cudaStream_t st) {
  return a.param_bf16 ? launch_infer_act<bf16>(a, act, st) : launch_infer_act<float>(a, act, st);
}

cudaError_t forward_res(const FwdArgs& a, const void* noise, int rows_per_sample, cudaStream_t st) {
  if (!a.identity) return forward(a, st);
  const cudaError_t e = launch_stats(a, nullptr, st);
  if (e != cudaSuccess) return e;
  const void* ptrs[3] = {a.x, a.y, a.identity};
  const int vec = vec_ok(a.c, ptrs, 3) ? kEwVec : 1;
  dim3 block, grid;
  ew_config(a.m, a.c, vec, &block, &grid);
  const ResTransformKernel k = res_transform_kernel(vec, noise != nullptr);
  if (!k) return kNoKernel;
  k<<<grid, block, 0, st>>>(static_cast<const bf16*>(a.x), static_cast<const bf16*>(a.identity), static_cast<const bf16*>(noise),
                            static_cast<bf16*>(a.y), a.save_mean, a.save_invstd, a.weight, a.bias, rows_per_sample, a.m, a.c);
  return cudaGetLastError();
}

cudaError_t backward_res(const BwdArgs& a, const void* noise, int rows_per_sample, cudaStream_t st) {
  if (!noise) {
    const cudaError_t e = launch_bwd_reduce(a, st);
    return e == cudaSuccess ? launch_elemt_of(a, static_cast<const bf16*>(a.dy), st) : e;
  }
  Scratch s = carve(a.scratch, a.c);
  dim3 block, grid;
  reduce_config(a.m, a.c, &block, &grid);
  const ResBwdReduceKernel kr = res_bwd_reduce_kernel();
  bf16* g = static_cast<bf16*>(a.dy_masked);
  kr<<<grid, block, 0, st>>>(static_cast<const bf16*>(a.x), static_cast<const bf16*>(a.dy), static_cast<const bf16*>(noise), a.save_mean,
                             a.save_invstd, s.sums, s.sums + a.c, a.grad_weight, a.grad_bias, s.staging, s.semaphores, g, rows_per_sample,
                             a.m, a.c);
  const cudaError_t e = cudaGetLastError();
  return e == cudaSuccess ? launch_elemt_of(a, g, st) : e;
}

template <typename P>
static cudaError_t launch_infer_res(const InferArgs& a, cudaStream_t st) {
  const void* ptrs[3] = {a.x, a.y, a.identity ? a.identity : a.x};
  const int vec = vec_ok(a.c, ptrs, 3) ? kEwVec : 1;
  dim3 block, grid;
  ew_config(a.m, a.c, vec, &block, &grid);
  const ResInferKernel<P> k = res_infer_kernel<P>(vec, a.identity != nullptr);
  if (!k) return kNoKernel;
  const InferParams& b = a.bn;
  k<<<grid, block, 0, st>>>(static_cast<const bf16*>(a.x), static_cast<const bf16*>(a.identity), static_cast<bf16*>(a.y),
                            static_cast<const P*>(b.running_mean), static_cast<const P*>(b.running_var), static_cast<const P*>(b.weight),
                            static_cast<const P*>(b.bias), b.eps, a.m, a.c);
  return cudaGetLastError();
}

cudaError_t infer_res(const InferArgs& a, cudaStream_t st) { return a.param_bf16 ? launch_infer_res<bf16>(a, st) : launch_infer_res<float>(a, st); }

static size_t sync_row_floats(int c) { return ((size_t)2 * c + 1 + 3) / 4 * 4; }
static size_t sync_rows_offset(int c) { return (scratch_bytes(c) + 15) / 16 * 16; }

size_t sync_scratch_bytes(int c, int world) { return sync_rows_offset(c) + (size_t)(world + 1) * sync_row_floats(c) * 4; }

SyncRows sync_rows(void* scratch, int c) {
  SyncRows r;
  r.row_floats = sync_row_floats(c);
  r.local = reinterpret_cast<float*>(static_cast<char*>(scratch) + sync_rows_offset(c));
  r.gathered = r.local + r.row_floats;
  r.sums = carve(scratch, c).sums;
  return r;
}

cudaError_t sync_stats(const FwdArgs& a, cudaStream_t st) {
  SyncRows r = sync_rows(a.scratch, a.c);
  if (a.m == 0) return cudaMemsetAsync(r.local, 0, ((size_t)2 * a.c + 1) * 4, st);
  return launch_stats(a, r.local, st);
}

cudaError_t sync_apply(const FwdArgs& a, int world, float* norm_fct, cudaStream_t st) {
  SyncRows r = sync_rows(a.scratch, a.c);
  k_bn_sync_merge<<<ceil_div(a.c, kEwThreads), kEwThreads, 0, st>>>(r.gathered, (int)r.row_floats, world, a.save_mean, a.save_invstd,
                                                                    norm_fct, a.running_mean, a.running_var, a.num_batches_tracked,
                                                                    a.momentum, a.eps, a.c);
  return a.m == 0 ? cudaGetLastError() : launch_transform(a, st);
}

cudaError_t sync_bwd_reduce(const BwdArgs& a, cudaStream_t st) {
  if (a.m == 0) {
    cudaMemsetAsync(carve(a.scratch, a.c).sums, 0, (size_t)2 * a.c * 4, st);
    cudaMemsetAsync(a.grad_weight, 0, (size_t)a.c * 4, st);
    cudaMemsetAsync(a.grad_bias, 0, (size_t)a.c * 4, st);
    return cudaGetLastError();
  }
  return launch_bwd_reduce(a, st);
}

cudaError_t sync_bwd_elemt(const BwdArgs& a, cudaStream_t st) { return a.m == 0 ? cudaSuccess : launch_bwd_elemt(a, st); }

static bn_cat::CatSegs cat_segs(const CatSegments& in) {
  bn_cat::CatSegs t{};
  int c = 0;
  for (int s = 0; s < in.n; s++) {
    t.ptr[s] = static_cast<const bf16*>(in.ptrs[s]);
    t.c0[s] = c;
    c += in.channels[s];
  }
  t.c0[in.n] = c;
  t.n = in.n;
  return t;
}

cudaError_t forward_cat(const CatSegments& in, const FwdArgs& a, cudaStream_t st) {
  const bn_cat::CatSegs segs = cat_segs(in);
  Scratch s = carve(a.scratch, a.c);
  dim3 block, grid;
  reduce_config(a.m, a.c, &block, &grid);
  block.x /= kStatsVec;
  StatsOut o{a.save_mean, a.save_invstd, a.running_mean, a.running_var, a.num_batches_tracked, a.momentum,
             (float)((double)a.m / (double)(a.m - 1)), a.eps};
  bn_cat::k_cat_stats<<<grid, block, stats_ring_bytes(block), st>>>(segs, o, s.staging, s.semaphores, a.m, a.c);
  cudaError_t e = cudaGetLastError();
  if (e != cudaSuccess) return e;
  ew_config(a.m, a.c, kEwVec, &block, &grid);
  bn_cat::k_cat_transform<<<grid, block, 0, st>>>(segs, static_cast<bf16*>(a.y), static_cast<uint8_t*>(a.mask), a.save_mean,
                                                  a.save_invstd, a.weight, a.bias, a.m, a.c);
  return cudaGetLastError();
}

cudaError_t backward_cat(const CatSegments& in, const BwdArgs& a, cudaStream_t st) {
  const bn_cat::CatSegs segs = cat_segs(in);
  Scratch s = carve(a.scratch, a.c);
  const void* ptrs[1] = {a.dy};
  const BwdReduceLaunch l = bwd_reduce_launch(a.m, a.c, kGradBits, false, false, ptrs, 1);
  if (l.vec != kBwdVec) return kNoKernel;
  bn_cat::k_cat_bwd_reduce<<<l.grid, l.block, l.smem, st>>>(segs, static_cast<const bf16*>(a.dy), static_cast<const uint8_t*>(a.mask),
                                                            a.save_mean, a.save_invstd, s.sums, s.sums + a.c, a.grad_weight,
                                                            a.grad_bias, s.staging, s.semaphores, a.m, a.c);
  cudaError_t e = cudaGetLastError();
  if (e != cudaSuccess) return e;
  dim3 block, grid;
  ew_config(a.m, a.c, kEwVec, &block, &grid);
  bn_cat::k_cat_bwd_elemt<<<grid, block, 0, st>>>(segs, static_cast<const bf16*>(a.dy), static_cast<const uint8_t*>(a.mask),
                                                  static_cast<bf16*>(a.dx), a.save_mean, a.save_invstd, a.weight, s.sums, s.sums + a.c,
                                                  (float)(1.0 / a.m), a.m, a.c);
  return cudaGetLastError();
}

template <typename P>
static cudaError_t launch_infer_cat(const CatSegments& in, const InferArgs& a, cudaStream_t st) {
  dim3 block, grid;
  ew_config(a.m, a.c, kEwVec, &block, &grid);
  const InferParams& b = a.bn;
  bn_cat::k_cat_infer<P><<<grid, block, 0, st>>>(cat_segs(in), static_cast<bf16*>(a.y), static_cast<const P*>(b.running_mean),
                                                 static_cast<const P*>(b.running_var), static_cast<const P*>(b.weight),
                                                 static_cast<const P*>(b.bias), b.eps, a.m, a.c);
  return cudaGetLastError();
}

cudaError_t infer_cat(const CatSegments& in, const InferArgs& a, cudaStream_t st) {
  return a.param_bf16 ? launch_infer_cat<bf16>(in, a, st) : launch_infer_cat<float>(in, a, st);
}

cudaError_t forward_slice(const FwdArgs& a, int ldy, cudaStream_t st) {
  const cudaError_t e = launch_stats(a, nullptr, st);
  if (e != cudaSuccess) return e;
  dim3 block, grid;
  ew_config(a.m, a.c, kEwVec, &block, &grid);
  bn_slice::k_slice_transform<<<grid, block, 0, st>>>(static_cast<const bf16*>(a.x), static_cast<bf16*>(a.y), ldy,
                                                      static_cast<uint8_t*>(a.mask), a.save_mean, a.save_invstd, a.weight, a.bias,
                                                      a.m, a.c);
  return cudaGetLastError();
}

cudaError_t backward_slice(const BwdArgs& a, int lddy, cudaStream_t st) {
  Scratch s = carve(a.scratch, a.c);
  const void* ptrs[2] = {a.x, a.dy};
  const BwdReduceLaunch l = bwd_reduce_launch(a.m, a.c, kGradBits, false, false, ptrs, 2);
  if (l.vec != kBwdVec) return kNoKernel;
  bn_slice::k_slice_bwd_reduce<<<l.grid, l.block, l.smem, st>>>(static_cast<const bf16*>(a.x), static_cast<const bf16*>(a.dy), lddy,
                                                                static_cast<const uint8_t*>(a.mask), a.save_mean, a.save_invstd, s.sums,
                                                                s.sums + a.c, a.grad_weight, a.grad_bias, s.staging, s.semaphores, a.m,
                                                                a.c);
  cudaError_t e = cudaGetLastError();
  if (e != cudaSuccess) return e;
  dim3 block, grid;
  ew_config(a.m, a.c, kEwVec, &block, &grid);
  bn_slice::k_slice_bwd_elemt<<<grid, block, 0, st>>>(static_cast<const bf16*>(a.dy), lddy, static_cast<const uint8_t*>(a.mask),
                                                      static_cast<const bf16*>(a.x), static_cast<bf16*>(a.dx), a.save_mean, a.save_invstd,
                                                      a.weight, s.sums, s.sums + a.c, (float)(1.0 / a.m), a.m, a.c);
  return cudaGetLastError();
}

template <typename P>
static cudaError_t launch_infer_slice(const InferArgs& a, int ldy, cudaStream_t st) {
  dim3 block, grid;
  ew_config(a.m, a.c, kEwVec, &block, &grid);
  const InferParams& b = a.bn;
  bn_slice::k_slice_infer<P><<<grid, block, 0, st>>>(static_cast<const bf16*>(a.x), static_cast<bf16*>(a.y), ldy,
                                                     static_cast<const P*>(b.running_mean), static_cast<const P*>(b.running_var),
                                                     static_cast<const P*>(b.weight), static_cast<const P*>(b.bias), b.eps, a.m, a.c);
  return cudaGetLastError();
}

cudaError_t infer_slice(const InferArgs& a, int ldy, cudaStream_t st) {
  return a.param_bf16 ? launch_infer_slice<bf16>(a, ldy, st) : launch_infer_slice<float>(a, ldy, st);
}

size_t shuffle_mask_bytes(int m, int c) { return (size_t)m * bn_shuffle::mask_row_bytes(c); }

static dim3 shuffle_tiles(int m, int c) { return dim3(ceil_div(m, bn_shuffle::kTile), ceil_div(c, bn_shuffle::kTile), 1); }

cudaError_t forward_shuffle(const FwdArgs& a, const FwdArgs* b, const void* x1, int x1_stride, int hw, cudaStream_t st) {
  const cudaError_t e = b ? launch_stats_dual(a, *b, st) : launch_stats(a, nullptr, st);
  if (e != cudaSuccess) return e;
  const bn_shuffle::Geometry g{a.m, a.c, hw, static_cast<const bf16*>(x1), x1_stride};
  const bn_shuffle::SavedStats sa{a.save_mean, a.save_invstd, a.weight, a.bias};
  const bf16* t = static_cast<const bf16*>(a.x);
  bf16* y = static_cast<bf16*>(a.y);
  uint8_t* mask = static_cast<uint8_t*>(a.mask);
  if (b) {
    const bn_shuffle::SavedStats sb{b->save_mean, b->save_invstd, b->weight, b->bias};
    bn_shuffle::k_shuffle_transform<true><<<shuffle_tiles(a.m, a.c), kEwThreads, 0, st>>>(t, static_cast<const bf16*>(b->x), y, mask,
                                                                                           static_cast<uint8_t*>(b->mask), sa, sb, g);
  } else {
    bn_shuffle::k_shuffle_transform<false><<<shuffle_tiles(a.m, a.c), kEwThreads, 0, st>>>(t, nullptr, y, mask, nullptr, sa, sa, g);
  }
  return cudaGetLastError();
}

cudaError_t backward_shuffle(const BwdArgs& a, const BwdArgs* b, cudaStream_t st) {
  Scratch s = carve(a.scratch, a.c);
  auto site = [](const BwdArgs& x, float* sum_xmu, float* staging) {
    return bn_shuffle::BwdSite{static_cast<const bf16*>(x.x), static_cast<const uint8_t*>(x.mask), x.save_mean, x.save_invstd, x.weight,
                               x.grad_weight, x.grad_bias, sum_xmu, staging, static_cast<bf16*>(x.dx)};
  };
  const bn_shuffle::BwdSite sa = site(a, s.sums + a.c, s.staging);
  const bn_shuffle::BwdSite sb = b ? site(*b, dual_sum_xmu2(a.scratch, a.c), dual_staging(a.scratch, a.c)) : sa;
  const bf16* dy = static_cast<const bf16*>(a.dy);
  dim3 block, grid;
  reduce_config(a.m, a.c, &block, &grid);
  if (b) bn_shuffle::k_shuffle_bwd_reduce<true><<<grid, block, 0, st>>>(dy, sa, sb, s.semaphores, a.m, a.c);
  else bn_shuffle::k_shuffle_bwd_reduce<false><<<grid, block, 0, st>>>(dy, sa, sb, s.semaphores, a.m, a.c);
  const cudaError_t e = cudaGetLastError();
  if (e != cudaSuccess) return e;
  ew_config(a.m, a.c, 1, &block, &grid);
  const float norm_fct = (float)(1.0 / a.m);
  if (b) bn_shuffle::k_shuffle_bwd_elemt<true><<<grid, block, 0, st>>>(dy, sa, sb, norm_fct, a.m, a.c);
  else bn_shuffle::k_shuffle_bwd_elemt<false><<<grid, block, 0, st>>>(dy, sa, sb, norm_fct, a.m, a.c);
  return cudaGetLastError();
}

template <typename P>
static cudaError_t launch_infer_shuffle(const InferArgs& a, const void* x1, int x1_stride, int hw, cudaStream_t st) {
  auto stats = [](const InferParams& q) {
    return bn_shuffle::RunningStats<P>{static_cast<const P*>(q.running_mean), static_cast<const P*>(q.running_var),
                                       static_cast<const P*>(q.weight), static_cast<const P*>(q.bias), q.eps};
  };
  const bn_shuffle::Geometry g{a.m, a.c, hw, static_cast<const bf16*>(x1), x1_stride};
  const bn_shuffle::RunningStats<P> sa = stats(a.bn);
  const bf16* t = static_cast<const bf16*>(a.x);
  bf16* y = static_cast<bf16*>(a.y);
  if (a.dual)
    bn_shuffle::k_shuffle_infer<true, P><<<shuffle_tiles(a.m, a.c), kEwThreads, 0, st>>>(t, static_cast<const bf16*>(a.identity), y, sa,
                                                                                          stats(a.ds), g);
  else
    bn_shuffle::k_shuffle_infer<false, P><<<shuffle_tiles(a.m, a.c), kEwThreads, 0, st>>>(t, nullptr, y, sa, sa, g);
  return cudaGetLastError();
}

cudaError_t infer_shuffle(const InferArgs& a, const void* x1, int x1_stride, int hw, cudaStream_t st) {
  return a.param_bf16 ? launch_infer_shuffle<bf16>(a, x1, x1_stride, hw, st) : launch_infer_shuffle<float>(a, x1, x1_stride, hw, st);
}

}
}
```

ant-ray_b200/csrc/norm_kernels.cuh:

```cuda
#pragma once
#include <cuda_bf16.h>
#include <cuda_runtime.h>
#include <stdint.h>

#include <type_traits>

namespace b200c {
namespace bn {

constexpr int kMaxBlock = 512;
constexpr int kParallelLoads = 4;
constexpr int kElemsPerThread = 16;
constexpr int kTileW = 32;
constexpr int kMaxHBlock = 128;
constexpr int kStatsVec = 4;
constexpr int kBwdVec = 4;
constexpr int kStatsStages = 4;
constexpr unsigned kBwdStages = 3;
constexpr unsigned kBwdStagesWide = 2;
__host__ __device__ constexpr unsigned bwd_ring_stages(int ops) { return ops >= 3 ? kBwdStagesWide : kBwdStages; }
__host__ __device__ constexpr int bwd_ring_operands(bool y, bool dy2, bool dual) { return 2 + dy2 + y + dual; }
constexpr int kEwThreads = 256;
constexpr int kEwVec = 8;

// ... 41 lines not shown
#pragma unroll
      for (int k = 0; k < V; k++) {
        shmem_mean[address_base + k] = mean[k];
        shmem_m2n[address_base + k] = m2n[k];
        shmem_count[address_base + k] = count[k];
      }
    }
    __syncthreads();
    if (threadIdx.y < offset && threadIdx.y + offset < blockDim.y) {
      auto address = address_base + offset * block_x;
#pragma unroll
      for (int k = 0; k < V; k++) {
        auto count_new = shmem_count[address + k];
        auto mean_new = shmem_mean[address + k];
        auto m2n_new = shmem_m2n[address + k];
        welford_merge_element<false>(count[k], mean[k], m2n[k], count_new, mean_new, m2n_new);
      }
    }
  }
}

template <int V>
__device__ __forceinline__ void merge_block_vertical_backward(float (&sum_dy)[V], float (&sum_dy_xmu)[V], float* shmem_sum_dy,
                                                              float* shmem_sum_dy_xmu) {
  const int block_x = blockDim.x * V;
  auto address_base = threadIdx.x * V + threadIdx.y * block_x;
#pragma unroll
  for (int offset = blockDim.y / 2; offset > 0; offset >>= 1) {
    if (threadIdx.y < offset * 2) {
#pragma unroll
      for (int k = 0; k < V; k++) {
        shmem_sum_dy[address_base + k] = sum_dy[k];
        shmem_sum_dy_xmu[address_base + k] = sum_dy_xmu[k];
      }
    }
    __syncthreads();
    if (threadIdx.y < offset && threadIdx.y + offset < blockDim.y) {
      auto address = address_base + offset * block_x;
#pragma unroll
      for (int k = 0; k < V; k++) {
        sum_dy[k] += shmem_sum_dy[address + k];
        sum_dy_xmu[k] += shmem_sum_dy_xmu[address + k];
      }
    }
  }
}

__device__ __forceinline__ void merge_block_vertical_backward(float& sum_dy, float& sum_dy_xmu, float* shmem_sum_dy,
                                                              float* shmem_sum_dy_xmu) {
  float a[1] = {sum_dy}, b[1] = {sum_dy_xmu};
  merge_block_vertical_backward<1>(a, b, shmem_sum_dy, shmem_sum_dy_xmu);
  sum_dy = a[0];
  sum_dy_xmu = b[0];
}

struct StatsOut {
  float* save_mean;
  float* save_invstd;
  float* running_mean;
  float* running_var;
  long long* num_batches_tracked;
  float momentum, bessel, eps;
};

__device__ __forceinline__ void finish_stats(const StatsOut& o, int c, float mean_th, float m2_th, int count_th) {
  const float mean = mean_th;
  const float var = m2_th / count_th;
  const float momentum = o.momentum;
  const float unbiased_var = var * o.bessel;
  o.save_mean[c] = mean;
  o.running_mean[c] = __fmaf_rn(mean, momentum, __fmul_rn(1 - momentum, o.running_mean[c]));
  o.running_var[c] = __fmaf_rn(unbiased_var, momentum, __fmul_rn(1 - momentum, o.running_var[c]));
  o.save_invstd[c] = rsqrtf(var + o.eps);
}

template <int V, typename Finish>
__device__ __forceinline__ void bn_stats_body(const bf16* __restrict__ input, volatile float* staging_data, int* semaphores,
                                              const int reduction_size, const int stride, Finish finish) {
  constexpr int PARALLEL_LOADS = kParallelLoads;
  float x_mean[PARALLEL_LOADS][V];
  float m_2_n[PARALLEL_LOADS][V];
  int count[PARALLEL_LOADS];
#pragma unroll
  for (int i = 0; i < PARALLEL_LOADS; i++) {
#pragma unroll
    for (int k = 0; k < V; k++) {
      x_mean[i][k] = 0.f;
      m_2_n[i][k] = 0.f;
    }
    count[i] = 0;
  }

  int inner_loop_stride = blockDim.y * gridDim.y;
  int m_offset = blockIdx.y * blockDim.y + threadIdx.y;
  int c_offset = (blockIdx.x * blockDim.x + threadIdx.x) * V;
  int loop_count = 1 + (reduction_size - 1) / (inner_loop_stride * PARALLEL_LOADS);
  const bool c_valid = c_offset < stride;

  auto update = [&](int j, const BVec<V>* xv) {
    float x_math[V];
    float x_count_inv;
    float is_valid;
    if (c_valid && m_offset < reduction_size) {
      const BVec<V> x = *xv;
#pragma unroll
      for (int k = 0; k < V; k++) x_math[k] = __bfloat162float(x.v[k]);
      count[j]++;
      x_count_inv = float(1) / count[j];
      is_valid = float(1);
    } else {
#pragma unroll
      for (int k = 0; k < V; k++) x_math[k] = float(0);
      x_count_inv = float(0);
      is_valid = float(0);
    }
    m_offset += inner_loop_stride;
#pragma unroll
    for (int k = 0; k < V; k++) {
      float delta0 = x_math[k] - x_mean[j][k];
      x_mean[j][k] = __fmaf_rn(delta0, x_count_inv, x_mean[j][k]);
      float delta1 = x_math[k] - x_mean[j][k];
      m_2_n[j][k] = __fmaf_rn(__fmul_rn(delta0, delta1), is_valid, m_2_n[j][k]);
    }
  };

  if constexpr (V == 1) {
    for (int i = 0; i < loop_count; i++) {
      BVec<V> xv[PARALLEL_LOADS];
#pragma unroll
      for (int j = 0; j < PARALLEL_LOADS; j++) {
        const int m = m_offset + j * inner_loop_stride;
        if (c_valid && m < reduction_size) xv[j] = *reinterpret_cast<const BVec<V>*>(input + ((size_t)m * stride + c_offset));
      }
#pragma unroll
      for (int j = 0; j < PARALLEL_LOADS; j++) update(j, &xv[j]);
    }
  } else {
    constexpr unsigned D = kStatsStages;
    const int threads = blockDim.x * blockDim.y;
    BVec<V>* ring = reinterpret_cast<BVec<V>*>(ring_smem()) + threadIdx.y * blockDim.x + threadIdx.x;
    const int first_row = m_offset;
    auto issue = [&](unsigned it) {
      BVec<V>* slot = ring + (it % D) * PARALLEL_LOADS * threads;
      int m = first_row + (int)it * PARALLEL_LOADS * inner_loop_stride;
#pragma unroll
      for (int j = 0; j < PARALLEL_LOADS; j++, m += inner_loop_stride)
        if (c_valid && m < reduction_size) cp_async<sizeof(BVec<V>)>(slot + j * threads, input + ((size_t)m * stride + c_offset));
      cp_async_commit();
    };
#pragma unroll
    for (unsigned it = 0; it < D - 1; it++) issue(it);
    for (unsigned i = 0; i < (unsigned)loop_count; i++) {
      issue(i + D - 1);
      cp_async_wait<D - 1>();
      const BVec<V>* slot = ring + (i % D) * PARALLEL_LOADS * threads;
#pragma unroll
      for (int j = 0; j < PARALLEL_LOADS; j++) update(j, slot + j * threads);
    }
  }
  float mean_th[V], m2_th[V];
  int count_th[V];
#pragma unroll
  for (int k = 0; k < V; k++) {
    count_th[k] = count[0];
    mean_th[k] = x_mean[0][k];
    m2_th[k] = m_2_n[0][k];
#pragma unroll
    for (int j = 1; j < PARALLEL_LOADS; j++) welford_merge_element<true>(count_th[k], mean_th[k], m2_th[k], count[j], x_mean[j][k], m_2_n[j][k]);
  }

  __shared__ float shmem_mean[kMaxBlock];
  __shared__ float shmem_m2n[kMaxBlock];
  __shared__ int shmem_count[kMaxBlock];
  welford_merge_block_vertical<V>(count_th, mean_th, m2_th, shmem_count, shmem_mean, shmem_m2n);

  if (gridDim.y > 1) {
    volatile float* staging_mean = staging_data;
    volatile float* staging_m2n = &staging_data[stride * gridDim.y];
    volatile int* staging_count = reinterpret_cast<volatile int*>(&staging_m2n[stride * gridDim.y]);
    int address_base = c_offset + blockIdx.y * stride;
    if (threadIdx.y == 0 && c_valid) {
#pragma unroll
      for (int k = 0; k < V; k++) {
        staging_mean[address_base + k] = mean_th[k];
        staging_m2n[address_base + k] = m2_th[k];
        staging_count[address_base + k] = count_th[k];
      }
    }
    __threadfence();
    __syncthreads();
    __shared__ bool is_last_block_done;
    if (threadIdx.x == 0 && threadIdx.y == 0) {
      int old = atomicAdd(&semaphores[blockIdx.x], 1);
      is_last_block_done = (old == (gridDim.y - 1));
      if (is_last_block_done) semaphores[blockIdx.x] = 0;
    }
    __syncthreads();
    if (is_last_block_done) {
#pragma unroll
      for (int k = 0; k < V; k++) {
        count_th[k] = 0;
        mean_th[k] = float(0.0);
        m2_th[k] = float(0.0);
      }
      for (int y = threadIdx.y; y < gridDim.y; y += blockDim.y) {
        address_base = c_offset + y * stride;
#pragma unroll
        for (int k = 0; k < V; k++) {
          int count_new = c_valid ? staging_count[address_base + k] : 0;
          float mean_new = c_valid ? staging_mean[address_base + k] : float(0.0);
          float m2n_new = c_valid ? staging_m2n[address_base + k] : float(0.0);
          welford_merge_element<false>(count_th[k], mean_th[k], m2_th[k], count_new, mean_new, m2n_new);
        }
      }
      welford_merge_block_vertical<V>(count_th, mean_th, m2_th, shmem_count, shmem_mean, shmem_m2n);
      if (threadIdx.y == 0 && c_valid)
#pragma unroll
        for (int k = 0; k < V; k++) finish(c_offset + k, mean_th[k], m2_th[k], count_th[k]);
    }
  } else {
    if (blockIdx.y == 0 && threadIdx.y == 0 && c_valid)
#pragma unroll
      for (int k = 0; k < V; k++) finish(c_offset + k, mean_th[k], m2_th[k], count_th[k]);
  }
}

template <int V>
__global__ void __launch_bounds__(kMaxBlock / V) k_bn_stats(const bf16* __restrict__ input, StatsOut o, volatile float* staging_data,
                                                            int* semaphores, const int reduction_size, const int stride) {
  if (o.num_batches_tracked && blockIdx.x == 0 && blockIdx.y == 0 && threadIdx.x == 0 && threadIdx.y == 0)
    *o.num_batches_tracked += 1;
  bn_stats_body<V>(input, staging_data, semaphores, reduction_size, stride,
                   [&](int c, float mean, float m2n, int count) { finish_stats(o, c, mean, m2n, count); });
}

template <int V>
__global__ void __launch_bounds__(kMaxBlock / V) k_bn_stats_dual(const bf16* __restrict__ input0, const bf16* __restrict__ input1,
                                                                 StatsOut o0, StatsOut o1, volatile float* staging0,
                                                                 volatile float* staging1, int* semaphores, const int reduction_size,
                                                                 const int stride) {
  const bool z = blockIdx.z != 0;
  const StatsOut o{z ? o1.save_mean : o0.save_mean, z ? o1.save_invstd : o0.save_invstd, z ? o1.running_mean : o0.running_mean,
                   z ? o1.running_var : o0.running_var, z ? o1.num_batches_tracked : o0.num_batches_tracked,
                   z ? o1.momentum : o0.momentum, z ? o1.bessel : o0.bessel, z ? o1.eps : o0.eps};
  if (o.num_batches_tracked && blockIdx.x == 0 && blockIdx.y == 0 && threadIdx.x == 0 && threadIdx.y == 0)
    *o.num_batches_tracked += 1;
  bn_stats_body<V>(z ? input1 : input0, z ? staging1 : staging0, semaphores + (z ? gridDim.x : 0), reduction_size, stride,
                   [&](int c, float mean, float m2n, int count) { finish_stats(o, c, mean, m2n, count); });
}


template <int V>
__global__ void __launch_bounds__(kMaxBlock / V) k_bn_sync_stats(const bf16* __restrict__ input, float* __restrict__ local,
                                                                 const float eps, volatile float* staging_data, int* semaphores,
                                                                 const int reduction_size, const int stride) {
  if (blockIdx.x == 0 && blockIdx.y == 0 && threadIdx.x == 0 && threadIdx.y == 0) local[2 * stride] = (float)reduction_size;
  bn_stats_body<V>(input, staging_data, semaphores, reduction_size, stride, [&](int c, float mean, float m2n, int count) {
    const float var = m2n / count;
    local[c] = mean;
    local[stride + c] = (var != 0.f || eps != 0.f) ? (float)(1.0 / sqrt((double)var + (double)eps)) : 0.f;
  });
}

__global__ void __launch_bounds__(kEwThreads) k_bn_sync_merge(const float* __restrict__ rows, const int row_stride, const int world,
                                                              float* __restrict__ save_mean, float* __restrict__ save_invstd,
                                                              float* __restrict__ norm_fct, float* __restrict__ running_mean,
                                                              float* __restrict__ running_var, long long* num_batches_tracked,
                                                              const float momentum, const float eps, const int stride) {
  const int i = blockIdx.x * blockDim.x + threadIdx.x;
  if (i == 0) {
    long long total = 0;
    for (int j = 0; j < world; j++) {
      const float count = rows[(size_t)j * row_stride + 2 * stride];
      if (count >= 1.f) total += (int)count;
    }
    *norm_fct = 1.f / (float)total;
    if (num_batches_tracked) *num_batches_tracked += 1;
  }
  if (i >= stride) return;
  float avg = 0.f, var_n = 0.f;
  int n = 0;
  for (int j = 0; j < world; j++) {
    const float* row = rows + (size_t)j * row_stride;
    const float count = row[2 * stride];
    if (!(count >= 1.f)) continue;
    const float m = row[i];
    float v = __fdiv_rn(1.f, row[stride + i]);
    v = __fmaf_rn(v, v, -eps);
    const float nf = (float)n;
    const float factor = __fdiv_rn(1.f, __fadd_rn(nf, count));
    const float d = __fsub_rn(avg, m);
    const float t = __fmul_rn(__fmul_rn(__fmul_rn(__fmul_rn(d, d), nf), count), factor);
    var_n = __fadd_rn(var_n, __fmaf_rn(v, count, t));
    avg = __fmaf_rn(__fmul_rn(nf, factor), avg, __fmul_rn(__fmul_rn(count, factor), m));
    n = (int)__fadd_rn(nf, count);
  }
  save_mean[i] = avg;
  save_invstd[i] = __fdiv_rn(1.f, __fsqrt_rn(__fadd_rn(__fdiv_rn(var_n, (float)n), eps)));
  running_mean[i] = __fmaf_rn(avg, momentum, __fmul_rn(1 - momentum, running_mean[i]));
  const float unbiased_var = __fdiv_rn(var_n, (float)(n - 1));
  running_var[i] = __fmaf_rn(unbiased_var, momentum, __fmul_rn(1 - momentum, running_var[i]));
}

enum Tail { kTailNone, kTailRelu, kTailAddRelu, kTailBnAddRelu };
constexpr int kTails = 4;

template <int V, Tail TAIL>
__global__ void __launch_bounds__(kEwThreads) k_bn_transform(const bf16* __restrict__ input, const bf16* __restrict__ identity,
                                                             bf16* __restrict__ out, uint8_t* __restrict__ mask,
                                                             const float* __restrict__ mean, const float* __restrict__ inv_std,
                                                             const float* __restrict__ weight, const float* __restrict__ shift,
                                                             const float* __restrict__ mean2, const float* __restrict__ inv_std2,
                                                             const float* __restrict__ weight2, const float* __restrict__ shift2,
                                                             const int reduction_size, const int stride) {
  static_assert(V == 1 || V == 8, "a thread writes a whole mask byte (V = 8) or one bit of a ballot (V = 1)");
  constexpr bool BN2 = TAIL == kTailBnAddRelu;
  const int c0 = (blockIdx.x * blockDim.x + threadIdx.x) * V;
  if (c0 >= stride) return;
  float m_c[V], inv_std_c[V], w_c[V], s_c[V], m2_c[V], inv_std2_c[V], w2_c[V], s2_c[V];
#pragma unroll
  for (int j = 0; j < V; j++) {
    m_c[j] = mean[c0 + j];
    inv_std_c[j] = inv_std[c0 + j];
    w_c[j] = weight[c0 + j];
    s_c[j] = shift[c0 + j];
    if (BN2) {
      m2_c[j] = mean2[c0 + j];
      inv_std2_c[j] = inv_std2[c0 + j];
      w2_c[j] = weight2[c0 + j];
      s2_c[j] = shift2[c0 + j];
    }
  }
  const unsigned lane = (threadIdx.x + threadIdx.y * blockDim.x) % 32;
  const unsigned group = 0xffu << (lane & ~7u);
  const int row_step = blockDim.y * gridDim.y;
  for (int m = blockIdx.y * blockDim.y + threadIdx.y; m < reduction_size; m += row_step) {
    const int a = m * stride + c0;
    const BVec<V> xv = *reinterpret_cast<const BVec<V>*>(input + a);
    BVec<V> zv;
    if (TAIL == kTailAddRelu || BN2) zv = *reinterpret_cast<const BVec<V>*>(identity + a);
    BVec<V> yv;
    unsigned bits = 0;
#pragma unroll
    for (int j = 0; j < V; j++) {
      auto tmp = w_c[j] * (__bfloat162float(xv.v[j]) - m_c[j]) * inv_std_c[j] + s_c[j];
      if (TAIL == kTailAddRelu || BN2) {
        if (BN2) zv.v[j] = __float2bfloat16(w2_c[j] * (__bfloat162float(zv.v[j]) - m2_c[j]) * inv_std2_c[j] + s2_c[j]);
        const bf16 r = __float2bfloat16(__bfloat162float(__float2bfloat16(tmp)) + __bfloat162float(zv.v[j]));
        yv.v[j] = __bfloat162float(r) <= 0.f ? __float2bfloat16(0.f) : r;
      } else if (TAIL == kTailRelu) {
        yv.v[j] = tmp <= 0.f ? __float2bfloat16(0.f) : __float2bfloat16(tmp);
      } else {
        yv.v[j] = __float2bfloat16(tmp);
      }
      bits |= (unsigned)!(__bfloat162float(yv.v[j]) <= 0.f) << j;
    }
    *reinterpret_cast<BVec<V>*>(out + a) = yv;
    if (TAIL != kTailNone && mask) {
      if (V == 1) bits = (__ballot_sync(group, bits) >> (lane & ~7u)) & 0xffu;
      if (V == 8 || lane % 8 == 0) mask[a >> 3] = (uint8_t)bits;
    }
  }
}

struct PoolDims {
  int h, w, oh, ow;
};
constexpr uint8_t kPoolNoGrad = 0xff;

template <int V>
__global__ void __launch_bounds__(kEwThreads) k_bn_pool_fwd(const bf16* __restrict__ input, bf16* __restrict__ out,
                                                            uint8_t* __restrict__ argmax, const float* __restrict__ mean,
                                                            const float* __restrict__ inv_std, const float* __restrict__ weight,
                                                            const float* __restrict__ shift, const PoolDims d, const int pooled_rows,
                                                            const int stride) {
  const int c0 = (blockIdx.x * blockDim.x + threadIdx.x) * V;
  if (c0 >= stride) return;
  float m_c[V], inv_std_c[V], w_c[V], s_c[V];
#pragma unroll
  for (int j = 0; j < V; j++) {
    m_c[j] = mean[c0 + j];
    inv_std_c[j] = inv_std[c0 + j];
    w_c[j] = weight[c0 + j];
    s_c[j] = shift[c0 + j];
  }
  const int row_step = blockDim.y * gridDim.y;
  for (int p = blockIdx.y * blockDim.y + threadIdx.y; p < pooled_rows; p += row_step) {
    const int pw = p % d.ow, ph = (p / d.ow) % d.oh, n = p / (d.ow * d.oh);
    float best[V];
    uint8_t pos[V];
#pragma unroll
    for (int j = 0; j < V; j++) {
      best[j] = -INFINITY;
      pos[j] = 0;
    }
    for (int ih = max(2 * ph - 1, 0); ih < min(2 * ph + 2, d.h); ih++) {
      for (int iw = max(2 * pw - 1, 0); iw < min(2 * pw + 2, d.w); iw++) {
        const BVec<V> xv = *reinterpret_cast<const BVec<V>*>(input + ((size_t)(n * d.h + ih) * d.w + iw) * stride + c0);
        const uint8_t at = (ih - 2 * ph + 1) * 3 + (iw - 2 * pw + 1);
#pragma unroll
        for (int j = 0; j < V; j++) {
          const auto tmp = w_c[j] * (__bfloat162float(xv.v[j]) - m_c[j]) * inv_std_c[j] + s_c[j];
          const float y = __bfloat162float(tmp <= 0.f ? __float2bfloat16(0.f) : __float2bfloat16(tmp));
          if (y > best[j] || isnan(y)) {
            best[j] = y;
            pos[j] = at;
          }
        }
      }
    }
    BVec<V> yv;
    struct alignas(V) {
      uint8_t v[V];
    } av;
#pragma unroll
    for (int j = 0; j < V; j++) {
      yv.v[j] = __float2bfloat16(best[j]);
      av.v[j] = best[j] <= 0.f ? kPoolNoGrad : pos[j];
    }
    const size_t a = (size_t)p * stride + c0;
    *reinterpret_cast<BVec<V>*>(out + a) = yv;
    *reinterpret_cast<decltype(av)*>(argmax + a) = av;
  }
}

__device__ __forceinline__ bf16 pool_grad(const bf16* __restrict__ dpool, const uint8_t* __restrict__ argmax, const PoolDims& d,
                                          const int m, const int c, const int stride) {
  const int iw = m % d.w, ih = (m / d.w) % d.h, n = m / (d.w * d.h);
  const int ph0 = ih >> 1, ph1 = min((ih + 1) >> 1, d.oh - 1);
  const int pw0 = iw >> 1, pw1 = min((iw + 1) >> 1, d.ow - 1);
  const int o = ((n * d.oh + ph0) * d.ow + pw0) * stride + c;
  const int dr = (ph1 - ph0) * d.ow * stride, dc = (pw1 - pw0) * stride;
  const uint8_t a[4] = {argmax[o], argmax[o + dc], argmax[o + dr], argmax[o + dr + dc]};
  const bf16 v[4] = {dpool[o], dpool[o + dc], dpool[o + dr], dpool[o + dr + dc]};
  const int at = (ih - 2 * ph0 + 1) * 3 + (iw - 2 * pw0 + 1);
  if (ph0 == ph1 && pw0 == pw1) return a[0] == at ? v[0] : __float2bfloat16(0.f);
  float sum = 0.f;
  if (a[0] == at) sum += __bfloat162float(v[0]);
  if (pw1 != pw0 && a[1] == at - 2) sum += __bfloat162float(v[1]);
  if (ph1 != ph0 && a[2] == at - 6) sum += __bfloat162float(v[2]);
  if (ph1 != ph0 && pw1 != pw0 && a[3] == at - 8) sum += __bfloat162float(v[3]);
  return __float2bfloat16(sum);
}

__device__ __forceinline__ bf16 relu_grad(bf16 dy, bf16 y) { return __bfloat162float(y) <= 0.f ? __float2bfloat16(0.f) : dy; }
__device__ __forceinline__ bf16 relu_grad_bit(bf16 dy, unsigned bit) { return bit ? dy : __float2bfloat16(0.f); }
__device__ __forceinline__ bf16 add_grads(bf16 a, bf16 b) { return __float2bfloat16(__bfloat162float(a) + __bfloat162float(b)); }

enum GradSrc { kGradMasked, kGradY, kGradBits, kGradDy, kGradPool };
constexpr int kGradSrcs = 5;

template <GradSrc G, bool DUAL>
__global__ void __launch_bounds__(kMaxBlock) k_bn_bwd_reduce(const bf16* __restrict__ input, const bf16* __restrict__ grad_output,
                                const bf16* __restrict__ grad_output2, const bf16* __restrict__ output,
                                const uint8_t* __restrict__ mask, bf16* __restrict__ masked, const float* __restrict__ mean,
                                const float* __restrict__ inv_std, float* __restrict__ sum_dy_o, float* __restrict__ sum_dy_xmu_o,
                                float* __restrict__ grad_weight, float* __restrict__ grad_bias, volatile float* staging_data,
                                int* semaphores, const PoolDims pool, const bf16* __restrict__ input2,
                                const float* __restrict__ mean2, const float* __restrict__ inv_std2, float* __restrict__ sum_dy_xmu2_o,
                                float* __restrict__ grad_weight2, float* __restrict__ grad_bias2, const int reduction_size,
                                const int stride, const int vec) {
  static_assert(G != kGradMasked, "the reduce kernel computes g");
  constexpr bool BITS = G == kGradBits;
  constexpr bool POOL = G == kGradPool;
  constexpr int PARALLEL_LOADS = kParallelLoads;
  __shared__ float shmem_sum_dy[kMaxBlock];
  __shared__ float shmem_sum_dy_xmu[kMaxBlock];
  __shared__ bool is_last_block_done;

  auto body = [&](auto vec_c) {
    constexpr int V = decltype(vec_c)::value;
    float sum_dy[PARALLEL_LOADS][V];
    float sum_dy_xmu[PARALLEL_LOADS][V];
    float sum_dy_xmu2[PARALLEL_LOADS][V];
#pragma unroll
    for (int i = 0; i < PARALLEL_LOADS; i++) {
#pragma unroll
      for (int k = 0; k < V; k++) {
        sum_dy[i][k] = float(0);
        sum_dy_xmu[i][k] = float(0);
        sum_dy_xmu2[i][k] = float(0);
      }
    }
    int inner_loop_stride = blockDim.y * gridDim.y;
    int m_offset = blockIdx.y * blockDim.y + threadIdx.y;
    int c_offset = (blockIdx.x * blockDim.x + threadIdx.x) * V;
    if (c_offset >= stride || m_offset >= reduction_size) return;

    int loop_count = 1 + (reduction_size - 1) / (inner_loop_stride * PARALLEL_LOADS);
    int address_base = m_offset * stride + c_offset;
    int address_increment = inner_loop_stride * stride;
    float r_mean[V], factor[V], r_mean2[V];
#pragma unroll
    for (int k = 0; k < V; k++) {
      r_mean[k] = mean[c_offset + k];
      factor[k] = inv_std[c_offset + k];
      r_mean2[k] = DUAL ? mean2[c_offset + k] : 0.f;
    }

    auto consume = [&](int j, const BVec<V>* dy_p, const BVec<V>* dy2_p, const BVec<V>* y_p, uint8_t mask_byte, const BVec<V>* x_p,
                       const BVec<V>* x2_p) {
      float x_input[V], x_input2[V], x_grad_output[V];
      if (m_offset < reduction_size) {
        const unsigned bits = BITS ? mask_byte >> (address_base & 7) : 0u;
        BVec<V> gv;
#pragma unroll
        for (int k = 0; k < V; k++) {
          const bf16 dy = !POOL && grad_output2 ? add_grads(dy_p->v[k], dy2_p->v[k]) : dy_p->v[k];
          gv.v[k] = BITS ? relu_grad_bit(dy, (bits >> k) & 1u) : G == kGradY ? relu_grad(dy, y_p->v[k]) : dy;
          x_input[k] = __bfloat162float(x_p->v[k]);
          x_input2[k] = DUAL ? __bfloat162float(x2_p->v[k]) : 0.f;
          x_grad_output[k] = __bfloat162float(gv.v[k]);
        }
        if (masked) *reinterpret_cast<BVec<V>*>(masked + address_base) = gv;
      } else {
#pragma unroll
        for (int k = 0; k < V; k++) {
          x_input[k] = float(0);
          x_input2[k] = float(0);
          x_grad_output[k] = float(0);
        }
      }
      m_offset += inner_loop_stride;
      address_base += address_increment;
#pragma unroll
      for (int k = 0; k < V; k++) {
        sum_dy[j][k] += x_grad_output[k];
        sum_dy_xmu[j][k] = __fmaf_rn(x_grad_output[k], x_input[k] - r_mean[k], sum_dy_xmu[j][k]);
        if (DUAL) sum_dy_xmu2[j][k] = __fmaf_rn(x_grad_output[k], x_input2[k] - r_mean2[k], sum_dy_xmu2[j][k]);
      }
    };

    if constexpr (V == 1) {
      for (int i = 0; i < loop_count; i++) {
        BVec<V> dy_v[PARALLEL_LOADS], dy2_v[PARALLEL_LOADS], y_v[PARALLEL_LOADS], x_v[PARALLEL_LOADS], x2_v[PARALLEL_LOADS];
        uint8_t mask_v[PARALLEL_LOADS];
#pragma unroll
        for (int j = 0; j < PARALLEL_LOADS; j++) {
          if (m_offset + j * inner_loop_stride < reduction_size) {
            const int a = address_base + j * address_increment;
            if (POOL) dy_v[j].v[0] = pool_grad(grad_output, mask, pool, m_offset + j * inner_loop_stride, c_offset, stride);
            else dy_v[j].v[0] = grad_output[a];
            if (grad_output2) dy2_v[j].v[0] = grad_output2[a];
            if (BITS) mask_v[j] = mask[a >> 3];
            else if (G == kGradY) y_v[j].v[0] = output[a];
            x_v[j].v[0] = input[a];
            if (DUAL) x2_v[j].v[0] = input2[a];
          }
        }
#pragma unroll
        for (int j = 0; j < PARALLEL_LOADS; j++) consume(j, &dy_v[j], &dy2_v[j], &y_v[j], mask_v[j], &x_v[j], &x2_v[j]);
      }
    } else {
      const int ops = bwd_ring_operands(G == kGradY, grad_output2 != nullptr, DUAL);
      auto ring_walk = [&](auto stages_c) {
        constexpr unsigned D = decltype(stages_c)::value;
        const int threads = blockDim.x * blockDim.y;
        const int op_dy2 = 2, op_y = op_dy2 + (grad_output2 != nullptr), op_x2 = op_y + (G == kGradY);
        BVec<V>* ring = reinterpret_cast<BVec<V>*>(ring_smem()) + threadIdx.y * blockDim.x + threadIdx.x;
        auto stage = [&](unsigned it) { return ring + (it % D) * ops * PARALLEL_LOADS * threads; };
        const int first_row = m_offset;
        const int iteration_rows = PARALLEL_LOADS * inner_loop_stride;
        auto issue = [&](unsigned it) {
          BVec<V>* slot = stage(it);
          int m = first_row + (int)it * iteration_rows;
#pragma unroll
          for (int j = 0; j < PARALLEL_LOADS; j++, m += inner_loop_stride, slot += threads) {
            if (m < reduction_size) {
              const size_t a = (size_t)m * stride + c_offset;
              cp_async<sizeof(BVec<V>)>(slot, grad_output + a);
              cp_async<sizeof(BVec<V>)>(slot + PARALLEL_LOADS * threads, input + a);
              if (grad_output2) cp_async<sizeof(BVec<V>)>(slot + op_dy2 * PARALLEL_LOADS * threads, grad_output2 + a);
              if (G == kGradY) cp_async<sizeof(BVec<V>)>(slot + op_y * PARALLEL_LOADS * threads, output + a);
              if (DUAL) cp_async<sizeof(BVec<V>)>(slot + op_x2 * PARALLEL_LOADS * threads, input2 + a);
            }
          }
          cp_async_commit();
        };
        uint8_t mask_next[PARALLEL_LOADS];
        auto load_mask = [&](unsigned it) {
          int m = first_row + (int)it * iteration_rows;
#pragma unroll
          for (int j = 0; j < PARALLEL_LOADS; j++, m += inner_loop_stride)
            if (m < reduction_size) mask_next[j] = mask[((size_t)m * stride + c_offset) >> 3];
        };
        if (BITS) load_mask(0);
#pragma unroll
        for (unsigned it = 0; it < D - 1; it++) issue(it);
        for (unsigned i = 0; i < (unsigned)loop_count; i++) {
          issue(i + D - 1);
          uint8_t mask_v[PARALLEL_LOADS];
#pragma unroll
          for (int j = 0; j < PARALLEL_LOADS; j++) mask_v[j] = mask_next[j];
          if (BITS) load_mask(i + 1);
          cp_async_wait<D - 1>();
          const BVec<V>* slot = stage(i);
#pragma unroll
          for (int j = 0; j < PARALLEL_LOADS; j++, slot += threads)
            consume(j, slot, slot + op_dy2 * PARALLEL_LOADS * threads, slot + op_y * PARALLEL_LOADS * threads, mask_v[j],
                    slot + PARALLEL_LOADS * threads, slot + op_x2 * PARALLEL_LOADS * threads);
        }
      };
      if (DUAL || bwd_ring_stages(ops) == kBwdStagesWide) ring_walk(std::integral_constant<unsigned, kBwdStagesWide>{});
      else ring_walk(std::integral_constant<unsigned, kBwdStages>{});
    }

    float sum_dy_th[V], sum_dy_xmu_th[V], sum_dy_xmu2_th[V];
#pragma unroll
    for (int k = 0; k < V; k++) {
#pragma unroll
      for (int j = 1; j < PARALLEL_LOADS; j++) {
        sum_dy[0][k] += sum_dy[j][k];
        sum_dy_xmu[0][k] += sum_dy_xmu[j][k];
        if (DUAL) sum_dy_xmu2[0][k] += sum_dy_xmu2[j][k];
      }
      sum_dy_th[k] = sum_dy[0][k];
      sum_dy_xmu_th[k] = sum_dy_xmu[0][k];
      sum_dy_xmu2_th[k] = sum_dy_xmu2[0][k];
    }

    auto merge = [&]() {
      merge_block_vertical_backward<V>(sum_dy_th, sum_dy_xmu_th, shmem_sum_dy, shmem_sum_dy_xmu);
      if (DUAL) {
        __syncthreads();
        float unused[V] = {};
        merge_block_vertical_backward<V>(sum_dy_xmu2_th, unused, shmem_sum_dy, shmem_sum_dy_xmu);
      }
    };
    merge();

    auto write_sums = [&]() {
#pragma unroll
      for (int k = 0; k < V; k++) {
        const int c = c_offset + k;
        grad_bias[c] = sum_dy_th[k];
        grad_weight[c] = sum_dy_xmu_th[k] * factor[k];
        sum_dy_o[c] = sum_dy_th[k];
        sum_dy_xmu_o[c] = sum_dy_xmu_th[k];
        if (DUAL) {
          grad_bias2[c] = sum_dy_th[k];
          grad_weight2[c] = sum_dy_xmu2_th[k] * inv_std2[c];
          sum_dy_xmu2_o[c] = sum_dy_xmu2_th[k];
        }
      }
    };
    if (gridDim.y > 1) {
      volatile float* staging_sum_dy = staging_data;
      volatile float* staging_sum_dy_xmu = &staging_data[stride * gridDim.y];
      volatile float* staging_sum_dy_xmu2 = &staging_data[2 * stride * gridDim.y];
      address_base = c_offset + blockIdx.y * stride;
      if (threadIdx.y == 0 && c_offset < stride) {
#pragma unroll
        for (int k = 0; k < V; k++) {
          staging_sum_dy[address_base + k] = sum_dy_th[k];
          staging_sum_dy_xmu[address_base + k] = sum_dy_xmu_th[k];
          if (DUAL) staging_sum_dy_xmu2[address_base + k] = sum_dy_xmu2_th[k];
        }
      }
      __threadfence();
      __syncthreads();
      if (threadIdx.x == 0 && threadIdx.y == 0) {
        int old = atomicAdd(&semaphores[blockIdx.x], 1);
        is_last_block_done = (old == (gridDim.y - 1));
        if (is_last_block_done) semaphores[blockIdx.x] = 0;
      }
      __syncthreads();
      if (is_last_block_done) {
#pragma unroll
        for (int k = 0; k < V; k++) {
          sum_dy_th[k] = float(0.0);
          sum_dy_xmu_th[k] = float(0.0);
          sum_dy_xmu2_th[k] = float(0.0);
        }
        for (int y = threadIdx.y; y < gridDim.y; y += blockDim.y) {
          address_base = c_offset + y * stride;
#pragma unroll
          for (int k = 0; k < V; k++) {
            sum_dy_th[k] += (c_offset < stride ? staging_sum_dy[address_base + k] : float(0.0));
            sum_dy_xmu_th[k] += (c_offset < stride ? staging_sum_dy_xmu[address_base + k] : float(0.0));
            if (DUAL) sum_dy_xmu2_th[k] += (c_offset < stride ? staging_sum_dy_xmu2[address_base + k] : float(0.0));
          }
        }
        merge();
        if (threadIdx.y == 0 && c_offset < stride) write_sums();
      }
    } else {
      if (blockIdx.y == 0 && threadIdx.y == 0 && c_offset < stride) write_sums();
    }
  };
  if constexpr (POOL) body(std::integral_constant<int, 1>{});
  else if (vec == kBwdVec) body(std::integral_constant<int, kBwdVec>{});
  else body(std::integral_constant<int, 1>{});
}

template <int V, GradSrc G, bool FCT_PTR, bool DUAL>
__global__ void __launch_bounds__(kEwThreads) k_bn_bwd_elemt(const bf16* __restrict__ grad_output, const bf16* __restrict__ grad_output2,
                                                             const bf16* __restrict__ output, const uint8_t* __restrict__ mask,
                                                             const bf16* __restrict__ input, bf16* __restrict__ grad_input,
                                                             const float* __restrict__ mean, const float* __restrict__ inv_std,
                                                             const float* __restrict__ weight, const float* __restrict__ sum_dy,
                                                             const float* __restrict__ sum_dy_xmu,
                                                             const float* __restrict__ norm_fct_ptr, const float norm_fct_value,
                                                             const bf16* __restrict__ input2, bf16* __restrict__ grad_input2,
                                                             const float* __restrict__ mean2, const float* __restrict__ inv_std2,
                                                             const float* __restrict__ weight2, const float* __restrict__ sum_dy_xmu2,
                                                             const int reduction_size, const int stride) {
  static_assert(!DUAL || (G == kGradY || G == kGradBits), "a dual tail derives g from dy and the ReLU");
  const float norm_fct = FCT_PTR ? *norm_fct_ptr : norm_fct_value;
  const int c0 = (blockIdx.x * blockDim.x + threadIdx.x) * V;
  if (c0 >= stride) return;
  float m_c[V], m_dy_c[V], factor_1_c[V], factor_2_c[V];
  float m2_c[V], factor2_1_c[V], factor2_2_c[V];
#pragma unroll
  for (int j = 0; j < V; j++) {
    m_c[j] = mean[c0 + j];
    m_dy_c[j] = sum_dy[c0 + j] * norm_fct;
    factor_1_c[j] = inv_std[c0 + j];
    factor_2_c[j] = weight[c0 + j] * factor_1_c[j];
    factor_1_c[j] = factor_1_c[j] * factor_1_c[j] * sum_dy_xmu[c0 + j] * norm_fct;
    if (DUAL) {
      m2_c[j] = mean2[c0 + j];
      factor2_1_c[j] = inv_std2[c0 + j];
      factor2_2_c[j] = weight2[c0 + j] * factor2_1_c[j];
      factor2_1_c[j] = factor2_1_c[j] * factor2_1_c[j] * sum_dy_xmu2[c0 + j] * norm_fct;
    }
  }
  const int row_step = blockDim.y * gridDim.y;
  for (int m = blockIdx.y * blockDim.y + threadIdx.y; m < reduction_size; m += row_step) {
    const int a = m * stride + c0;
    const BVec<V> gv = *reinterpret_cast<const BVec<V>*>(grad_output + a);
    BVec<V> gv2, yv;
    if (G != kGradMasked && grad_output2) gv2 = *reinterpret_cast<const BVec<V>*>(grad_output2 + a);
    unsigned bits = 0;
    if (G == kGradY) yv = *reinterpret_cast<const BVec<V>*>(output + a);
    if (G == kGradBits) bits = mask[a >> 3] >> (a & 7);
    const BVec<V> xv = *reinterpret_cast<const BVec<V>*>(input + a);
    BVec<V> x2v, dxv, dx2v;
    if (DUAL) x2v = *reinterpret_cast<const BVec<V>*>(input2 + a);
#pragma unroll
    for (int j = 0; j < V; j++) {
      const bf16 dy = G != kGradMasked && grad_output2 ? add_grads(gv.v[j], gv2.v[j]) : gv.v[j];
      const float g = __bfloat162float(G == kGradMasked || G == kGradDy ? dy
                                       : G == kGradY ? relu_grad(dy, yv.v[j]) : relu_grad_bit(dy, (bits >> j) & 1u));
      dxv.v[j] = __float2bfloat16((g - m_dy_c[j] - (__bfloat162float(xv.v[j]) - m_c[j]) * factor_1_c[j]) * factor_2_c[j]);
      if (DUAL)
        dx2v.v[j] = __float2bfloat16((g - m_dy_c[j] - (__bfloat162float(x2v.v[j]) - m2_c[j]) * factor2_1_c[j]) * factor2_2_c[j]);
    }
    *reinterpret_cast<BVec<V>*>(grad_input + a) = dxv;
    if (DUAL) *reinterpret_cast<BVec<V>*>(grad_input2 + a) = dx2v;
  }
}

}
}
```

ant-ray_b200/csrc/norm_launch.h:

```cpp
#pragma once
#include <cuda_runtime.h>
#include <stddef.h>

namespace b200c {
namespace bn {

struct FwdArgs {
  const void* x;
  const void* identity;
  void* y;
  void* mask;
  bool relu;
  const float* weight;
  const float* bias;
  float* running_mean;
  float* running_var;
  long long* num_batches_tracked;
  float* save_mean;
  float* save_invstd;
  int m, c;
  float momentum, eps;
  void* scratch;
  void* argmax;
  int pool_h, pool_w;
};

struct BwdArgs {
  const void* dy;
  const void* dy2;
  const void* y;
  const void* mask;
  const void* x;
  void* dy_masked;
  void* dx;
  bool relu;
  const float* weight;
  const float* save_mean;
  const float* save_invstd;
  const float* norm_fct;
  float* grad_weight;
  float* grad_bias;
  int m, c;
  void* scratch;
  const void* argmax;
  int pool_h, pool_w;
};

constexpr int kMaxChannels = 1 << 17;

size_t scratch_bytes(int c);
cudaError_t forward(const FwdArgs& a, cudaStream_t s);
cudaError_t backward(const BwdArgs& a, cudaStream_t s);

size_t dual_scratch_bytes(int c);
cudaError_t forward_dual(const FwdArgs& a, const FwdArgs& b, cudaStream_t s);
cudaError_t backward_dual(const BwdArgs& a, const BwdArgs& b, cudaStream_t s);

struct SyncRows {
  float* local;
  float* gathered;
  size_t row_floats;
  float* sums;
};
size_t sync_scratch_bytes(int c, int world);
SyncRows sync_rows(void* scratch, int c);
cudaError_t sync_stats(const FwdArgs& a, cudaStream_t s);
cudaError_t sync_apply(const FwdArgs& a, int world, float* norm_fct, cudaStream_t s);
cudaError_t sync_bwd_reduce(const BwdArgs& a, cudaStream_t s);
cudaError_t sync_bwd_elemt(const BwdArgs& a, cudaStream_t s);
cudaError_t load_kernels();

struct InferParams {
  const void* weight;
  const void* bias;
  const void* running_mean;
  const void* running_var;
  float eps;
};
struct InferArgs {
  const void* x;
  const void* identity;
  void* y;
  InferParams bn;
  InferParams ds;
  bool dual, param_bf16;
  int m, c;
  int pool_h, pool_w;
};
cudaError_t infer(const InferArgs& a, cudaStream_t s);

bool act_ok(int act);
cudaError_t forward_act(const FwdArgs& a, int act, cudaStream_t s);
cudaError_t backward_act(const BwdArgs& a, const float* bias, int act, cudaStream_t s);
cudaError_t infer_act(const InferArgs& a, int act, cudaStream_t s);

cudaError_t forward_res(const FwdArgs& a, const void* noise, int rows_per_sample, cudaStream_t s);
cudaError_t backward_res(const BwdArgs& a, const void* noise, int rows_per_sample, cudaStream_t s);
cudaError_t infer_res(const InferArgs& a, cudaStream_t s);

constexpr int kMaxCatSegs = 64;
struct CatSegments {
  const void* const* ptrs;
  const int* channels;
  int n;
};
cudaError_t forward_cat(const CatSegments& segs, const FwdArgs& a, cudaStream_t s);
cudaError_t backward_cat(const CatSegments& segs, const BwdArgs& a, cudaStream_t s);
cudaError_t infer_cat(const CatSegments& segs, const InferArgs& a, cudaStream_t s);

cudaError_t forward_slice(const FwdArgs& a, int ldy, cudaStream_t s);
cudaError_t backward_slice(const BwdArgs& a, int lddy, cudaStream_t s);
cudaError_t infer_slice(const InferArgs& a, int ldy, cudaStream_t s);

size_t shuffle_mask_bytes(int m, int c);
cudaError_t forward_shuffle(const FwdArgs& a, const FwdArgs* b, const void* x1, int x1_stride, int hw, cudaStream_t s);
cudaError_t backward_shuffle(const BwdArgs& a, const BwdArgs* b, cudaStream_t s);
cudaError_t infer_shuffle(const InferArgs& a, const void* x1, int x1_stride, int hw, cudaStream_t s);

}
}
```

include/b200coll.h:

```cpp
#ifndef B200COLL_H_
#define B200COLL_H_

#include <stddef.h>
#include <stdint.h>

#ifdef __cplusplus
extern "C" {
#endif

#define B200C_VERSION 200
#define B200C_MAX_RANKS 8

typedef enum {
  B200C_INT8 = 0,
  B200C_UINT8 = 1,
  B200C_INT32 = 2,
  B200C_UINT32 = 3,
  B200C_INT64 = 4,
  B200C_UINT64 = 5,
  B200C_FLOAT16 = 6,
  B200C_FLOAT32 = 7,
  B200C_FLOAT64 = 8,
  B200C_BFLOAT16 = 9,
  B200C_NUM_DTYPES = 10
} b200c_dtype_t;

typedef enum {
  B200C_SUM = 0,
  B200C_PROD = 1,
  B200C_MAX = 2,
  B200C_MIN = 3,
  B200C_AVG = 4,
  B200C_NUM_OPS = 5
} b200c_redop_t;

typedef enum {
  B200C_ALGO_AUTO = 0,
  B200C_ALGO_ONESHOT = 1,
  B200C_ALGO_TWOSHOT = 2,
  B200C_ALGO_NVLS = 3,
  B200C_ALGO_NVLS_PIPE = 4,
  B200C_ALGO_LL = 5,
  B200C_ALGO_NVLS_LANES = 6,
  B200C_ALGO_NVLS_STREAMS = 7
} b200c_algo_t;

typedef enum {
  B200C_OK = 0,
  B200C_EINVAL = -1,
  B200C_ECUDA = -2,
  B200C_ESTATE = -3,
  B200C_EUNSUPPORTED = -4,
  B200C_ETIMEOUT = -5,
  B200C_EABORTED = -6,
  B200C_EMISMATCH = -7,
  B200C_ENOMEM = -8
} b200c_status_t;

typedef enum {
  B200C_SHARE_VMM_FD = 0,
  B200C_SHARE_LEGACY_IPC = 1
} b200c_share_mode_t;

typedef struct {
  uint32_t struct_size;
  int32_t share_mode;
  uint64_t staging_bytes;
  uint64_t symmetric_bytes;
  uint64_t p2p_slot_bytes;
  uint32_t p2p_slots;
  uint32_t max_blocks;
  uint64_t oneshot_max_bytes;
  uint64_t nvls_min_bytes;
  uint64_t nvls_pipe_min_bytes;
  uint64_t timeout_ms;
  uint64_t granule_bytes;
  uint64_t ll_max_bytes;
  uint64_t bcast_rounds_min_bytes;
  uint32_t nvls_blocks;
  uint32_t nvls_lanes;
  uint64_t lane_granule_bytes;
  uint64_t nvls_lanes_min_bytes;
  uint32_t nvls_unroll;
  uint32_t rounds_order;
  uint64_t nvls_streams_min_bytes;
  uint64_t nvls_streams_piece_bytes;
} b200c_config_t;

typedef struct {
  int32_t device;
  int32_t sm_count;
  int32_t cc_major, cc_minor;
  int32_t vmm_supported;
  int32_t posix_fd_supported;
  int32_t multicast_supported;
  int32_t reserved;
  uint64_t total_mem;
} b200c_props_t;

typedef struct {
  int32_t share_mode;
  int32_t fd;
  uint64_t arena_bytes;
  uint64_t layout_hash;
  int32_t pid;
  int32_t device_uuid_lo;
  uint8_t ipc[64];
} b200c_export_t;

typedef struct b200c_comm b200c_comm_t;
typedef void* b200c_stream_t;

int b200c_version(void);
const char* b200c_last_error(void);
const char* b200c_status_string(int status);
size_t b200c_dtype_size(int dtype);
int b200c_device_props(int device, b200c_props_t* out);
void b200c_default_config(b200c_config_t* cfg);

int b200c_comm_create(int rank, int world, int device, const b200c_config_t* cfg, b200c_comm_t** out);
int b200c_comm_export(b200c_comm_t* comm, b200c_export_t* out);
int b200c_comm_import(b200c_comm_t* comm, int peer, const b200c_export_t* peer_export);
int b200c_comm_mc_create(b200c_comm_t* comm, int* fd_out);
int b200c_comm_mc_import(b200c_comm_t* comm, int fd);
int b200c_comm_mc_add_device(b200c_comm_t* comm);
int b200c_comm_mc_bind(b200c_comm_t* comm);
int b200c_comm_mc_disable(b200c_comm_t* comm);
int b200c_comm_ready(b200c_comm_t* comm);
int b200c_comm_abort(b200c_comm_t* comm);
int b200c_comm_destroy(b200c_comm_t* comm);
int b200c_comm_check(b200c_comm_t* comm);
int b200c_comm_rank(const b200c_comm_t* comm);
int b200c_comm_world(const b200c_comm_t* comm);
int b200c_comm_has_multicast(const b200c_comm_t* comm);
uint64_t b200c_comm_seq(const b200c_comm_t* comm);

void* b200c_comm_symmetric_base(b200c_comm_t* comm);
uint64_t b200c_comm_symmetric_bytes(const b200c_comm_t* comm);

int b200c_pool_bind(b200c_comm_t* comm);
void* b200c_pool_malloc(size_t size, int device, void* stream);
void b200c_pool_free(void* ptr, size_t size, int device, void* stream);


int b200c_allreduce(b200c_comm_t* comm, const void* send, void* recv, size_t count, int dtype,
                    int op, int algo, b200c_stream_t stream);

int b200c_allreduce_scaled(b200c_comm_t* comm, const void* send, void* recv, size_t count, int dtype,
                           int wire_dtype, float scale, int algo, b200c_stream_t stream);

int b200c_reduce(b200c_comm_t* comm, const void* send, void* recv, size_t count, int dtype, int op,
                 int root, b200c_stream_t stream);

int b200c_broadcast(b200c_comm_t* comm, void* buf, size_t count, int dtype, int root,
                    b200c_stream_t stream);

int b200c_allgather(b200c_comm_t* comm, const void* send, void* const* recv_ptrs, size_t count,
                    int dtype, b200c_stream_t stream);

int b200c_reducescatter(b200c_comm_t* comm, const void* const* send_ptrs, void* recv, size_t count,
                        int dtype, int op, b200c_stream_t stream);

int b200c_reducescatter_scaled(b200c_comm_t* comm, const void* const* send_ptrs, void* recv, size_t count,
                               int dtype, int wire_dtype, float scale, b200c_stream_t stream);

int b200c_send(b200c_comm_t* comm, const void* buf, size_t bytes, int peer, b200c_stream_t stream);
int b200c_recv(b200c_comm_t* comm, void* buf, size_t bytes, int peer, b200c_stream_t stream);

int b200c_send_multi(b200c_comm_t* comm, const void* buf, size_t bytes, const int* peers, int npeers,
                     b200c_stream_t stream);
int b200c_recv_multi(b200c_comm_t* comm, void* buf, size_t bytes, int src, b200c_stream_t stream);

int b200c_barrier(b200c_comm_t* comm, b200c_stream_t stream);

int b200c_debug_fill_flags(b200c_comm_t* comm, uint32_t value);

size_t b200c_bn_scratch_bytes(int channels);
int b200c_bn_forward(const void* x, const void* identity, void* y, const float* weight, const float* bias,
                     float* running_mean, float* running_var, int64_t* num_batches_tracked, float* save_mean,
                     float* save_invstd, int m, int channels, float momentum, float eps, void* scratch,
                     b200c_stream_t stream);
int b200c_bn_forward_mask(const void* x, const void* identity, void* y, uint8_t* mask, const float* weight,
                          const float* bias, float* running_mean, float* running_var, int64_t* num_batches_tracked,
                          float* save_mean, float* save_invstd, int m, int channels, float momentum, float eps,
                          void* scratch, b200c_stream_t stream);
int b200c_bn_backward(const void* dy, const void* y, const void* x, void* dy_masked, void* dx, const float* weight,
                      const float* save_mean, const float* save_invstd, float* grad_weight, float* grad_bias, int m,
                      int channels, void* scratch, b200c_stream_t stream);
int b200c_bn_backward_mask(const void* dy, const void* dy2, const uint8_t* mask, const void* x, void* dy_masked, void* dx,
                           const float* weight, const float* save_mean, const float* save_invstd, float* grad_weight,
                           float* grad_bias, int m, int channels, void* scratch, b200c_stream_t stream);

size_t b200c_bn_dual_scratch_bytes(int channels);
int b200c_bn_forward_dual(const void* x, const void* x_ds, void* y, uint8_t* mask, const float* weight, const float* bias,
                          float* running_mean, float* running_var, int64_t* num_batches_tracked, float* save_mean,
                          float* save_invstd, float momentum, float eps, const float* weight_ds, const float* bias_ds,
                          float* running_mean_ds, float* running_var_ds, int64_t* num_batches_tracked_ds,
                          float* save_mean_ds, float* save_invstd_ds, float momentum_ds, float eps_ds, int m, int channels,
                          void* scratch, b200c_stream_t stream);
int b200c_bn_backward_dual(const void* dy, const void* dy2, const void* y, const uint8_t* mask, const void* x,
                           const void* x_ds, void* dx, void* dx_ds, const float* weight, const float* save_mean,
                           const float* save_invstd, float* grad_weight, float* grad_bias, const float* weight_ds,
                           const float* save_mean_ds, const float* save_invstd_ds, float* grad_weight_ds,
                           float* grad_bias_ds, int m, int channels, void* scratch, b200c_stream_t stream);

int b200c_bn_forward_pool(const void* x, void* y, uint8_t* argmax, const float* weight, const float* bias,
                          float* running_mean, float* running_var, int64_t* num_batches_tracked, float* save_mean,
                          float* save_invstd, int n, int h, int w, int channels, float momentum, float eps, void* scratch,
                          b200c_stream_t stream);
int b200c_bn_backward_pool(const void* dy, const uint8_t* argmax, const void* x, void* g, void* dx, const float* weight,
                           const float* save_mean, const float* save_invstd, float* grad_weight, float* grad_bias, int n,
                           int h, int w, int channels, void* scratch, b200c_stream_t stream);

int b200c_bn_infer(const void* x, const void* identity, void* y, const void* weight, const void* bias, const void* running_mean,
                   const void* running_var, int param_bf16, float eps, int m, int channels, b200c_stream_t stream);
int b200c_bn_infer_dual(const void* x, const void* x_ds, void* y, const void* weight, const void* bias, const void* running_mean,
                        const void* running_var, float eps, const void* weight_ds, const void* bias_ds, const void* running_mean_ds,
                        const void* running_var_ds, float eps_ds, int param_bf16, int m, int channels, b200c_stream_t stream);
int b200c_bn_infer_pool(const void* x, void* y, const void* weight, const void* bias, const void* running_mean,
                        const void* running_var, int param_bf16, float eps, int n, int h, int w, int channels,
                        b200c_stream_t stream);

typedef enum { B200C_ACT_RELU6 = 1, B200C_ACT_SILU = 2, B200C_ACT_HARDSWISH = 3 } b200c_act_t;
int b200c_bn_forward_act(const void* x, void* y, const float* weight, const float* bias, float* running_mean, float* running_var,
                         int64_t* num_batches_tracked, float* save_mean, float* save_invstd, int act, int m, int channels,
                         float momentum, float eps, void* scratch, b200c_stream_t stream);
int b200c_bn_backward_act(const void* dy, const void* x, void* g, void* dx, const float* weight, const float* bias, const float* save_mean,
                          const float* save_invstd, float* grad_weight, float* grad_bias, int act, int m, int channels, void* scratch,
                          b200c_stream_t stream);
int b200c_bn_infer_act(const void* x, void* y, const void* weight, const void* bias, const void* running_mean, const void* running_var,
                       int param_bf16, float eps, int act, int m, int channels, b200c_stream_t stream);

int b200c_bn_forward_res(const void* x, const void* identity, const void* noise, int rows_per_sample, void* y, const float* weight,
                         const float* bias, float* running_mean, float* running_var, int64_t* num_batches_tracked, float* save_mean,
                         float* save_invstd, int m, int channels, float momentum, float eps, void* scratch, b200c_stream_t stream);
int b200c_bn_backward_res(const void* dy, const void* noise, int rows_per_sample, const void* x, void* g, void* dx, const float* weight,
                          const float* save_mean, const float* save_invstd, float* grad_weight, float* grad_bias, int m, int channels,
                          void* scratch, b200c_stream_t stream);
int b200c_bn_infer_res(const void* x, const void* identity, void* y, const void* weight, const void* bias, const void* running_mean,
                       const void* running_var, int param_bf16, float eps, int m, int channels, b200c_stream_t stream);

int b200c_bn_forward_cat(const void* const* segs, const int* seg_channels, int nsegs, void* y, uint8_t* mask, const float* weight,
                         const float* bias, float* running_mean, float* running_var, int64_t* num_batches_tracked, float* save_mean,
                         float* save_invstd, int m, int channels, float momentum, float eps, void* scratch, b200c_stream_t stream);
int b200c_bn_backward_cat(const void* dy, const uint8_t* mask, const void* const* segs, const int* seg_channels, int nsegs, void* dx,
                          const float* weight, const float* save_mean, const float* save_invstd, float* grad_weight, float* grad_bias,
                          int m, int channels, void* scratch, b200c_stream_t stream);
int b200c_bn_infer_cat(const void* const* segs, const int* seg_channels, int nsegs, void* y, const void* weight, const void* bias,
                       const void* running_mean, const void* running_var, int param_bf16, float eps, int m, int channels,
                       b200c_stream_t stream);

int b200c_bn_forward_slice(const void* x, void* y, int ldy, uint8_t* mask, const float* weight, const float* bias, float* running_mean,
                           float* running_var, int64_t* num_batches_tracked, float* save_mean, float* save_invstd, int m, int channels,
                           float momentum, float eps, void* scratch, b200c_stream_t stream);
int b200c_bn_backward_slice(const void* dy, int lddy, const uint8_t* mask, const void* x, void* dx, const float* weight,
                            const float* save_mean, const float* save_invstd, float* grad_weight, float* grad_bias, int m, int channels,
                            void* scratch, b200c_stream_t stream);
int b200c_bn_infer_slice(const void* x, void* y, int ldy, const void* weight, const void* bias, const void* running_mean,
                         const void* running_var, int param_bf16, float eps, int m, int channels, b200c_stream_t stream);

size_t b200c_bn_shuffle_mask_bytes(int m, int channels);
int b200c_bn_forward_shuffle(const void* x1, int x1_stride, const void* u, uint8_t* mask_u, const float* weight_u, const float* bias_u,
                             float* running_mean_u, float* running_var_u, int64_t* num_batches_tracked_u, float* save_mean_u,
                             float* save_invstd_u, float momentum_u, float eps_u, const void* t, uint8_t* mask, const float* weight,
                             const float* bias, float* running_mean, float* running_var, int64_t* num_batches_tracked, float* save_mean,
                             float* save_invstd, float momentum, float eps, void* y, int n, int hw, int channels, void* scratch,
                             b200c_stream_t stream);
int b200c_bn_backward_shuffle(const void* dy, const void* u, const uint8_t* mask_u, void* du, const float* weight_u, const float* save_mean_u,
                              const float* save_invstd_u, float* grad_weight_u, float* grad_bias_u, const void* t, const uint8_t* mask,
                              void* dt, const float* weight, const float* save_mean, const float* save_invstd, float* grad_weight,
                              float* grad_bias, int m, int channels, void* scratch, b200c_stream_t stream);
int b200c_bn_infer_shuffle(const void* x1, int x1_stride, const void* u, const void* weight_u, const void* bias_u, const void* running_mean_u,
                           const void* running_var_u, float eps_u, const void* t, const void* weight, const void* bias,
                           const void* running_mean, const void* running_var, float eps, void* y, int param_bf16, int n, int hw,
                           int channels, b200c_stream_t stream);

size_t b200c_se_scratch_bytes(int n, int channels, int hw);
int b200c_se_pool(const void* x, void* pooled, int n, int channels, int hw, void* scratch, size_t scratch_bytes, b200c_stream_t stream);
int b200c_se_scale(const void* x, const void* s, void* y, int n, int channels, int hw, b200c_stream_t stream);
int b200c_se_backward_reduce(const void* dy, const void* x, void* ds, int n, int channels, int hw, void* scratch, size_t scratch_bytes,
                             b200c_stream_t stream);
int b200c_se_backward_elemt(const void* dy, const void* s, const void* gp, void* dx, int n, int channels, int hw,
                            b200c_stream_t stream);

size_t b200c_bn_sync_scratch_bytes(int channels, int world);
int b200c_bn_sync_forward(b200c_comm_t* comm, const void* x, const void* identity, void* y, uint8_t* mask, int relu,
                          const float* weight, const float* bias, float* running_mean, float* running_var,
                          int64_t* num_batches_tracked, float* save_mean, float* save_invstd, float* norm_fct, int m,
                          int channels, float momentum, float eps, void* scratch, b200c_stream_t stream);
int b200c_bn_sync_backward(b200c_comm_t* comm, const void* dy, const void* dy2, const void* y, const uint8_t* mask, int relu,
                           const void* x, void* dy_masked, void* dx, const float* weight, const float* save_mean,
                           const float* save_invstd, const float* norm_fct, float* grad_weight, float* grad_bias, int m,
                           int channels, void* scratch, b200c_stream_t stream);

uint64_t b200c_launch_count(void);

#ifdef __cplusplus
}
#endif
#endif
```

Measured before the change: 5568.

## Order BN elementwise pass rows to reuse L2 data left by stats pass

The batch-norm elementwise kernels (forward transform and backward elemt) now walk rows in an order chosen to match what the preceding reduction kernel touched last. Small tensors are walked in reverse so the most recently read rows are still in L2. When the reduction grid exceeds one resident wave, rows are visited by group in reverse and the second grid is capped at one wave. This is meant to cut HBM re-reads between the two passes, at the cost of extra index arithmetic per row, occupancy queries (cached) and a debug hook that reports the chosen walk.

```diff
diff --git a/ant-ray_b200/_native.py b/ant-ray_b200/_native.py
--- a/ant-ray_b200/_native.py
+++ b/ant-ray_b200/_native.py
@@ -90,6 +90,7 @@
     "b200c_barrier": (c_int, [c_void_p, c_void_p]),
     "b200c_debug_fill_flags": (c_int, [c_void_p, c_uint32]),
     "b200c_bn_scratch_bytes": (c_size_t, [c_int]),
+    "b200c_bn_last_walk": (c_int, []),
     "b200c_bn_forward": (c_int, [c_void_p] * 10 + [c_int, c_int, c_float, c_float, c_void_p, c_void_p]),
     "b200c_bn_forward_mask": (c_int, [c_void_p] * 11 + [c_int, c_int, c_float, c_float, c_void_p, c_void_p]),
     "b200c_bn_backward": (c_int, [c_void_p] * 10 + [c_int, c_int, c_void_p, c_void_p]),
diff --git a/ant-ray_b200/csrc/b200coll.cu b/ant-ray_b200/csrc/b200coll.cu
--- a/ant-ray_b200/csrc/b200coll.cu
+++ b/ant-ray_b200/csrc/b200coll.cu
@@ -1260,6 +1260,8 @@
   return channels < 1 || channels > bn::kMaxChannels || world < 1 || world > kMaxRanks ? 0 : bn::sync_scratch_bytes(channels, world);
 }
 
+extern "C" int b200c_bn_last_walk(void) { return bn::last_walk(); }
+
 static const char* bn_site(bool sync) { return sync ? "sync batch norm" : "batch norm"; }
 
 static int check_bn(const char* site, int min_m, int m, int c, const void* scratch, int relu, const void* mask, const void* residual,
diff --git a/ant-ray_b200/csrc/inst_norm.cu b/ant-ray_b200/csrc/inst_norm.cu
--- a/ant-ray_b200/csrc/inst_norm.cu
+++ b/ant-ray_b200/csrc/inst_norm.cu
@@ -1,5 +1,9 @@
 #include <algorithm>
+#include <climits>
 #include <initializer_list>
+#include <map>
+#include <mutex>
+#include <tuple>
 #include <type_traits>
 
 #include "norm_act.cuh"
@@ -84,6 +88,48 @@
   *grid = dim3(gx, gy, 1);
 }
 
+static int resident_blocks(const void* kernel, int threads, size_t smem) {
+  static std::mutex mu;
+  static std::map<std::tuple<int, const void*, int, size_t>, int> cache;
+  int dev = 0;
+  if (cudaGetDevice(&dev) != cudaSuccess) return 0;
+  const auto key = std::make_tuple(dev, kernel, threads, smem);
+  std::lock_guard<std::mutex> lock(mu);
+  const auto it = cache.find(key);
+  if (it != cache.end()) return it->second;
+  int per_sm = 0, sms = 0;
+  if (cudaOccupancyMaxActiveBlocksPerMultiprocessor(&per_sm, kernel, threads, smem) != cudaSuccess ||
+      cudaDeviceGetAttribute(&sms, cudaDevAttrMultiProcessorCount, dev) != cudaSuccess)
+    return 0;
+  return cache[key] = per_sm * sms;
+}
+
+constexpr size_t kMirrorMaxBytes = 64 << 20;
+static thread_local int g_last_walk = -1;
+static RowWalk rows_walk(int rows, bool falling) {
+  g_last_walk = falling ? kWalkFalling : kWalkRising;
+  return RowWalk{rows, rows, falling ? 1 : -1, 0};
+}
+static bool mirror_ok(int m, int c) { return (size_t)m * c * sizeof(bf16) <= kMirrorMaxBytes; }
+static RowWalk walk_after(const void* kernel, dim3 block, dim3 grid, size_t smem, int m, int c) {
+  const long long blocks = (long long)grid.x * grid.y * grid.z;
+  const int band = block.y * grid.y;
+  const long long span = (long long)ceil_div(m, band) * band;
+  if (grid.y > 1 && span <= INT_MAX && blocks > resident_blocks(kernel, block.x * block.y, smem)) {
+    g_last_walk = kWalkGroups;
+    return RowWalk{(int)span, (int)(span / grid.y), band, __builtin_ctz(block.y)};
+  }
+  return rows_walk(m, mirror_ok(m, c));
+}
+int last_walk() { return g_last_walk; }
+
+static void second_config(const void* kernel, const RowWalk& walk, int rows, int stride, int vec, dim3* block, dim3* grid) {
+  ew_config(rows, stride, vec, block, grid);
+  if (walk.band < 0) return;
+  const int wave = resident_blocks(kernel, block->x * block->y, 0) / (int)grid->x;
+  grid->y = std::max(1, std::min((int)grid->y, wave));
+}
+
 constexpr int kSemaphores = kMaxChannels / kTileW;
 constexpr size_t kSemaphoreBytes = (size_t)kSemaphores * 4;
 
@@ -116,14 +162,14 @@
 using SyncStatsKernel = void (*)(const bf16*, float*, float, volatile float*, int*, int, int);
 using StatsDualKernel = void (*)(const bf16*, const bf16*, StatsOut, StatsOut, volatile float*, volatile float*, int*, int, int);
 using TransformKernel = void (*)(const bf16*, const bf16*, bf16*, uint8_t*, const float*, const float*, const float*, const float*,
-                                 const float*, const float*, const float*, const float*, int, int);
+                                 const float*, const float*, const float*, const float*, RowWalk, int, int);
 using PoolFwdKernel = void (*)(const bf16*, bf16*, uint8_t*, const float*, const float*, const float*, const float*, PoolDims, int, int);
 using BwdReduceKernel = void (*)(const bf16*, const bf16*, const bf16*, const bf16*, const uint8_t*, bf16*, const float*, const float*,
                                  float*, float*, float*, float*, volatile float*, int*, PoolDims, const bf16*, const float*, const float*,
                                  float*, float*, float*, int, int, int);
 using BwdElemtKernel = void (*)(const bf16*, const bf16*, const bf16*, const uint8_t*, const bf16*, bf16*, const float*, const float*,
                                 const float*, const float*, const float*, const float*, float, const bf16*, bf16*, const float*,
-                                const float*, const float*, const float*, int, int);
+                                const float*, const float*, const float*, RowWalk, int, int);
 
 static StatsKernel stats_kernel(int vec) {
   return with_const<1, kStatsVec>(vec, [](auto v) -> StatsKernel { return k_bn_stats<decltype(v)::value>; });
@@ -296,38 +342,53 @@
 
 constexpr cudaError_t kNoKernel = cudaErrorInvalidDeviceFunction;
 
+struct StatsLaunch {
+  dim3 block, grid;
+  int vec;
+  size_t smem;
+};
+static StatsLaunch stats_launch(const FwdArgs& a) {
+  StatsLaunch l;
+  reduce_config(a.m, a.c, &l.block, &l.grid);
+  l.vec = vec_ok(a.c, &a.x, 1) ? kStatsVec : 1;
+  l.block.x /= l.vec;
+  l.smem = l.vec == kStatsVec ? stats_ring_bytes(l.block) : 0;
+  return l;
+}
+static RowWalk stats_walk(const FwdArgs& a, bool sync) {
+  const StatsLaunch l = stats_launch(a);
+  const void* k = sync ? (const void*)sync_stats_kernel(l.vec) : (const void*)stats_kernel(l.vec);
+  return walk_after(k, l.block, l.grid, l.smem, a.m, a.c);
+}
+
 static cudaError_t launch_stats(const FwdArgs& a, float* sync_row, cudaStream_t st) {
   Scratch s = carve(a.scratch, a.c);
-  dim3 block, grid;
-  reduce_config(a.m, a.c, &block, &grid);
-  const int vec = vec_ok(a.c, &a.x, 1) ? kStatsVec : 1;
-  block.x /= vec;
-  const size_t smem = vec == kStatsVec ? stats_ring_bytes(block) : 0;
+  const StatsLaunch l = stats_launch(a);
   const bf16* x = static_cast<const bf16*>(a.x);
   if (sync_row) {
-    const SyncStatsKernel k = sync_stats_kernel(vec);
+    const SyncStatsKernel k = sync_stats_kernel(l.vec);
     if (!k) return kNoKernel;
-    k<<<grid, block, smem, st>>>(x, sync_row, a.eps, s.staging, s.semaphores, a.m, a.c);
+    k<<<l.grid, l.block, l.smem, st>>>(x, sync_row, a.eps, s.staging, s.semaphores, a.m, a.c);
   } else {
-    const StatsKernel k = stats_kernel(vec);
+    const StatsKernel k = stats_kernel(l.vec);
     if (!k) return kNoKernel;
     StatsOut o{a.save_mean, a.save_invstd, a.running_mean, a.running_var, a.num_batches_tracked, a.momentum,
                (float)((double)a.m / (double)(a.m - 1)), a.eps};
-    k<<<grid, block, smem, st>>>(x, o, s.staging, s.semaphores, a.m, a.c);
+    k<<<l.grid, l.block, l.smem, st>>>(x, o, s.staging, s.semaphores, a.m, a.c);
   }
   return cudaGetLastError();
 }
 
-static cudaError_t launch_transform(const FwdArgs& a, cudaStream_t st) {
+static cudaError_t launch_transform(const FwdArgs& a, const RowWalk& walk, cudaStream_t st) {
   const void* ptrs[3] = {a.x, a.y, a.identity ? a.identity : a.x};
   const int vec = vec_ok(a.c, ptrs, 3) ? kEwVec : 1;
-  dim3 block, grid;
-  ew_config(a.m, a.c, vec, &block, &grid);
   const TransformKernel k = transform_kernel(vec, !a.relu ? kTailNone : a.identity ? kTailAddRelu : kTailRelu);
   if (!k) return kNoKernel;
+  dim3 block, grid;
+  second_config((const void*)k, walk, a.m, a.c, vec, &block, &grid);
   k<<<grid, block, 0, st>>>(static_cast<const bf16*>(a.x), static_cast<const bf16*>(a.identity), static_cast<bf16*>(a.y),
                             static_cast<uint8_t*>(a.mask), a.save_mean, a.save_invstd, a.weight, a.bias, nullptr, nullptr, nullptr,
-                            nullptr, a.m, a.c);
+                            nullptr, walk, a.m, a.c);
   return cudaGetLastError();
 }
 
@@ -338,10 +399,11 @@
   const int pooled_rows = a.m / (a.pool_h * a.pool_w) * d.oh * d.ow;
   const void* ptrs[3] = {a.x, a.y, a.argmax};
   const int vec = vec_ok(a.c, ptrs, 3) ? kEwVec : 1;
-  dim3 block, grid;
-  ew_config(pooled_rows, a.c, vec, &block, &grid);
   const PoolFwdKernel k = pool_fwd_kernel(vec);
   if (!k) return kNoKernel;
+  dim3 block, grid;
+  ew_config(pooled_rows, a.c, vec, &block, &grid);
+  g_last_walk = kWalkRising;
   k<<<grid, block, 0, st>>>(static_cast<const bf16*>(a.x), static_cast<bf16*>(a.y), static_cast<uint8_t*>(a.argmax), a.save_mean,
                             a.save_invstd, a.weight, a.bias, d, pooled_rows, a.c);
   return cudaGetLastError();
@@ -350,7 +412,7 @@
 cudaError_t forward(const FwdArgs& a, cudaStream_t st) {
   const cudaError_t e = launch_stats(a, nullptr, st);
   if (e != cudaSuccess) return e;
-  return a.pool_h ? launch_pool_fwd(a, st) : launch_transform(a, st);
+  return a.pool_h ? launch_pool_fwd(a, st) : launch_transform(a, stats_walk(a, false), st);
 }
 
 static GradSrc grad_src(const BwdArgs& a, bool reduced) {
@@ -360,11 +422,20 @@
   return a.mask ? kGradBits : kGradY;
 }
 
-static cudaError_t launch_bwd_reduce(const BwdArgs& a, cudaStream_t st) {
-  Scratch s = carve(a.scratch, a.c);
+static BwdReduceLaunch local_reduce_launch(const BwdArgs& a) {
   const GradSrc src = grad_src(a, false);
   const void* ptrs[5] = {a.x, a.dy, a.dy2 ? a.dy2 : a.dy, src == kGradY ? a.y : a.dy, a.dy_masked ? a.dy_masked : a.dy};
-  const BwdReduceLaunch l = bwd_reduce_launch(a.m, a.c, src, a.dy2 != nullptr, false, ptrs, 5);
+  return bwd_reduce_launch(a.m, a.c, src, a.dy2 != nullptr, false, ptrs, 5);
+}
+static RowWalk bwd_reduce_walk(const BwdArgs& a) {
+  const BwdReduceLaunch l = local_reduce_launch(a);
+  return walk_after((const void*)bwd_reduce_kernel(grad_src(a, false), false), l.block, l.grid, l.smem, a.m, a.c);
+}
+
+static cudaError_t launch_bwd_reduce(const BwdArgs& a, cudaStream_t st) {
+  Scratch s = carve(a.scratch, a.c);
+  const GradSrc src = grad_src(a, false);
+  const BwdReduceLaunch l = local_reduce_launch(a);
   const BwdReduceKernel k = bwd_reduce_kernel(src, false);
   if (!k) return kNoKernel;
   const void* mask = src == kGradPool ? a.argmax : a.mask;
@@ -381,14 +452,15 @@
   const void* g = src == kGradMasked ? a.dy_masked : a.dy;
   const void* ptrs[5] = {a.x, a.dx, g, a.dy2 && src != kGradMasked ? a.dy2 : a.dy, a.y};
   const int vec = vec_ok(a.c, ptrs, src == kGradY ? 5 : 4) ? kEwVec : 1;
-  dim3 block, grid;
-  ew_config(a.m, a.c, vec, &block, &grid);
   const BwdElemtKernel k = bwd_elemt_kernel(vec, src, a.norm_fct != nullptr, false);
   if (!k) return kNoKernel;
+  const RowWalk walk = bwd_reduce_walk(a);
+  dim3 block, grid;
+  second_config((const void*)k, walk, a.m, a.c, vec, &block, &grid);
   k<<<grid, block, 0, st>>>(static_cast<const bf16*>(g), static_cast<const bf16*>(a.dy2), static_cast<const bf16*>(a.y),
                             static_cast<const uint8_t*>(a.mask), static_cast<const bf16*>(a.x), static_cast<bf16*>(a.dx), a.save_mean,
                             a.save_invstd, a.weight, s.sums, s.sums + a.c, a.norm_fct, (float)(1.0 / a.m), nullptr, nullptr, nullptr,
-                            nullptr, nullptr, nullptr, a.m, a.c);
+                            nullptr, nullptr, nullptr, walk, a.m, a.c);
   return cudaGetLastError();
 }
 
@@ -402,22 +474,27 @@
 static float* dual_staging(void* scratch, int c) { return reinterpret_cast<float*>(static_cast<char*>(scratch) + dual_extra_offset(c)); }
 static float* dual_sum_xmu2(void* scratch, int c) { return dual_staging(scratch, c) + (size_t)3 * c * kMaxHBlock; }
 
+static StatsLaunch dual_stats_launch(const FwdArgs& a, const FwdArgs& b) {
+  StatsLaunch l;
+  reduce_config(a.m, a.c, &l.block, &l.grid);
+  const void* xs[2] = {a.x, b.x};
+  l.vec = vec_ok(a.c, xs, 2) ? kStatsVec : 1;
+  l.block.x /= l.vec;
+  l.grid.z = 2;
+  l.smem = l.vec == kStatsVec ? stats_ring_bytes(l.block) : 0;
+  return l;
+}
+
 static cudaError_t launch_stats_dual(const FwdArgs& a, const FwdArgs& b, cudaStream_t st) {
   Scratch s = carve(a.scratch, a.c);
-  dim3 block, grid;
-  reduce_config(a.m, a.c, &block, &grid);
-  const void* xs[2] = {a.x, b.x};
-  const int svec = vec_ok(a.c, xs, 2) ? kStatsVec : 1;
-  block.x /= svec;
-  grid.z = 2;
-  const size_t smem = svec == kStatsVec ? stats_ring_bytes(block) : 0;
-  const StatsDualKernel ks = stats_dual_kernel(svec);
+  const StatsLaunch l = dual_stats_launch(a, b);
+  const StatsDualKernel ks = stats_dual_kernel(l.vec);
   if (!ks) return kNoKernel;
   StatsOut oa{a.save_mean, a.save_invstd, a.running_mean, a.running_var, a.num_batches_tracked, a.momentum,
               (float)((double)a.m / (double)(a.m - 1)), a.eps};
   StatsOut ob{b.save_mean, b.save_invstd, b.running_mean, b.running_var, b.num_batches_tracked, b.momentum,
               (float)((double)b.m / (double)(b.m - 1)), b.eps};
-  ks<<<grid, block, smem, st>>>(static_cast<const bf16*>(a.x), static_cast<const bf16*>(b.x), oa, ob, s.staging,
+  ks<<<l.grid, l.block, l.smem, st>>>(static_cast<const bf16*>(a.x), static_cast<const bf16*>(b.x), oa, ob, s.staging,
                              dual_staging(a.scratch, a.c), s.semaphores, a.m, a.c);
   return cudaGetLastError();
 }
@@ -425,15 +502,17 @@
 cudaError_t forward_dual(const FwdArgs& a, const FwdArgs& b, cudaStream_t st) {
   const cudaError_t e = launch_stats_dual(a, b, st);
   if (e != cudaSuccess) return e;
-  dim3 block, grid;
   const void* ptrs[3] = {a.x, a.y, b.x};
   const int vec = vec_ok(a.c, ptrs, 3) ? kEwVec : 1;
-  ew_config(a.m, a.c, vec, &block, &grid);
   const TransformKernel kt = transform_kernel(vec, kTailBnAddRelu);
   if (!kt) return kNoKernel;
+  const StatsLaunch l = dual_stats_launch(a, b);
+  const RowWalk walk = walk_after((const void*)stats_dual_kernel(l.vec), l.block, l.grid, l.smem, a.m, a.c);
+  dim3 block, grid;
+  second_config((const void*)kt, walk, a.m, a.c, vec, &block, &grid);
   kt<<<grid, block, 0, st>>>(static_cast<const bf16*>(a.x), static_cast<const bf16*>(b.x), static_cast<bf16*>(a.y),
                              static_cast<uint8_t*>(a.mask), a.save_mean, a.save_invstd, a.weight, a.bias, b.save_mean, b.save_invstd,
-                             b.weight, b.bias, a.m, a.c);
+                             b.weight, b.bias, walk, a.m, a.c);
   return cudaGetLastError();
 }
 
@@ -453,14 +532,15 @@
   if (e != cudaSuccess) return e;
   const void* ptrs[7] = {a.x, a.dx, a.dy, a.dy2 ? a.dy2 : a.dy, b.x, b.dx, a.y};
   const int vec = vec_ok(a.c, ptrs, src == kGradY ? 7 : 6) ? kEwVec : 1;
-  dim3 block, grid;
-  ew_config(a.m, a.c, vec, &block, &grid);
   const BwdElemtKernel ke = bwd_elemt_kernel(vec, src, false, true);
   if (!ke) return kNoKernel;
+  const RowWalk walk = walk_after((const void*)kr, l.block, l.grid, l.smem, a.m, a.c);
+  dim3 block, grid;
+  second_config((const void*)ke, walk, a.m, a.c, vec, &block, &grid);
   ke<<<grid, block, 0, st>>>(static_cast<const bf16*>(a.dy), static_cast<const bf16*>(a.dy2), static_cast<const bf16*>(a.y),
                              static_cast<const uint8_t*>(a.mask), static_cast<const bf16*>(a.x), static_cast<bf16*>(a.dx), a.save_mean,
                              a.save_invstd, a.weight, s.sums, s.sums + a.c, nullptr, (float)(1.0 / a.m), static_cast<const bf16*>(b.x),
-                             static_cast<bf16*>(b.dx), b.save_mean, b.save_invstd, b.weight, sum2, a.m, a.c);
+                             static_cast<bf16*>(b.dx), b.save_mean, b.save_invstd, b.weight, sum2, walk, a.m, a.c);
   return cudaGetLastError();
 }
 
@@ -495,17 +575,17 @@
 
 cudaError_t infer(const InferArgs& a, cudaStream_t st) { return a.param_bf16 ? launch_infer<bf16>(a, st) : launch_infer<float>(a, st); }
 
-static cudaError_t launch_elemt_of(const BwdArgs& a, const bf16* g, cudaStream_t st) {
+static cudaError_t launch_elemt_of(const BwdArgs& a, const bf16* g, const RowWalk& walk, cudaStream_t st) {
   Scratch s = carve(a.scratch, a.c);
   const void* ptrs[3] = {a.x, a.dx, g};
   const int vec = vec_ok(a.c, ptrs, 3) ? kEwVec : 1;
-  dim3 block, grid;
-  ew_config(a.m, a.c, vec, &block, &grid);
   const BwdElemtKernel ke = bwd_elemt_kernel(vec, kGradMasked, false, false);
   if (!ke) return kNoKernel;
+  dim3 block, grid;
+  second_config((const void*)ke, walk, a.m, a.c, vec, &block, &grid);
   ke<<<grid, block, 0, st>>>(g, nullptr, nullptr, nullptr, static_cast<const bf16*>(a.x), static_cast<bf16*>(a.dx), a.save_mean,
                              a.save_invstd, a.weight, s.sums, s.sums + a.c, nullptr, (float)(1.0 / a.m), nullptr, nullptr, nullptr,
-                             nullptr, nullptr, nullptr, a.m, a.c);
+                             nullptr, nullptr, nullptr, walk, a.m, a.c);
   return cudaGetLastError();
 }
 
@@ -534,7 +614,7 @@
                              a.grad_weight, a.grad_bias, s.staging, s.semaphores, g, a.m, a.c);
   cudaError_t e = cudaGetLastError();
   if (e != cudaSuccess) return e;
-  return launch_elemt_of(a, g, st);
+  return launch_elemt_of(a, g, walk_after((const void*)kr, block, grid, 0, a.m, a.c), st);
 }
 
 template <typename P>
@@ -574,7 +654,7 @@
 cudaError_t backward_res(const BwdArgs& a, const void* noise, int rows_per_sample, cudaStream_t st) {
   if (!noise) {
     const cudaError_t e = launch_bwd_reduce(a, st);
-    return e == cudaSuccess ? launch_elemt_of(a, static_cast<const bf16*>(a.dy), st) : e;
+    return e == cudaSuccess ? launch_elemt_of(a, static_cast<const bf16*>(a.dy), bwd_reduce_walk(a), st) : e;
   }
   Scratch s = carve(a.scratch, a.c);
   dim3 block, grid;
@@ -585,7 +665,7 @@
                              a.save_invstd, s.sums, s.sums + a.c, a.grad_weight, a.grad_bias, s.staging, s.semaphores, g, rows_per_sample,
                              a.m, a.c);
   const cudaError_t e = cudaGetLastError();
-  return e == cudaSuccess ? launch_elemt_of(a, g, st) : e;
+  return e == cudaSuccess ? launch_elemt_of(a, g, walk_after((const void*)kr, block, grid, 0, a.m, a.c), st) : e;
 }
 
 template <typename P>
@@ -630,7 +710,7 @@
   k_bn_sync_merge<<<ceil_div(a.c, kEwThreads), kEwThreads, 0, st>>>(r.gathered, (int)r.row_floats, world, a.save_mean, a.save_invstd,
                                                                     norm_fct, a.running_mean, a.running_var, a.num_batches_tracked,
                                                                     a.momentum, a.eps, a.c);
-  return a.m == 0 ? cudaGetLastError() : launch_transform(a, st);
+  return a.m == 0 ? cudaGetLastError() : launch_transform(a, stats_walk(a, true), st);
 }
 
 cudaError_t sync_bwd_reduce(const BwdArgs& a, cudaStream_t st) {
diff --git a/ant-ray_b200/csrc/norm_kernels.cuh b/ant-ray_b200/csrc/norm_kernels.cuh
--- a/ant-ray_b200/csrc/norm_kernels.cuh
+++ b/ant-ray_b200/csrc/norm_kernels.cuh
@@ -367,6 +367,39 @@
   running_var[i] = __fmaf_rn(unbiased_var, momentum, __fmul_rn(1 - momentum, running_var[i]));
 }
 
+struct RowWalk {
+  int span;
+  int group;
+  int band;
+  int shift;
+  __device__ __forceinline__ void start(int t, int& g, int& r) const {
+    const int u = span - 1 - t;
+    g = u / group;
+    r = u - g * group;
+  }
+  __device__ __forceinline__ void next(int step, int& g, int& r) const {
+    r -= step;
+    while (r < 0 && g > 0) {
+      r += group;
+      g--;
+    }
+  }
+  __device__ __forceinline__ int row(int g, int r) const { return (r >> shift) * band + (g << shift) + (r & ((1 << shift) - 1)); }
+  template <typename F>
+  __device__ __forceinline__ void visit(int first, int step, int rows, F&& f) const {
+    if (band < 0) {
+      for (int m = first; m < rows; m += step) f(m);
+      return;
+    }
+    int g, r;
+    start(first, g, r);
+    for (int t = first; t < span; t += step, next(step, g, r)) {
+      const int m = row(g, r);
+      if (m < rows) f(m);
+    }
+  }
+};
+
 enum Tail { kTailNone, kTailRelu, kTailAddRelu, kTailBnAddRelu };
 constexpr int kTails = 4;
 
@@ -377,7 +410,7 @@
                                                              const float* __restrict__ weight, const float* __restrict__ shift,
                                                              const float* __restrict__ mean2, const float* __restrict__ inv_std2,
                                                              const float* __restrict__ weight2, const float* __restrict__ shift2,
-                                                             const int reduction_size, const int stride) {
+                                                             const RowWalk walk, const int reduction_size, const int stride) {
   static_assert(V == 1 || V == 8, "a thread writes a whole mask byte (V = 8) or one bit of a ballot (V = 1)");
   constexpr bool BN2 = TAIL == kTailBnAddRelu;
   const int c0 = (blockIdx.x * blockDim.x + threadIdx.x) * V;
@@ -399,7 +432,7 @@
   const unsigned lane = (threadIdx.x + threadIdx.y * blockDim.x) % 32;
   const unsigned group = 0xffu << (lane & ~7u);
   const int row_step = blockDim.y * gridDim.y;
-  for (int m = blockIdx.y * blockDim.y + threadIdx.y; m < reduction_size; m += row_step) {
+  walk.visit(blockIdx.y * blockDim.y + threadIdx.y, row_step, reduction_size, [&](const int m) {
     const int a = m * stride + c0;
     const BVec<V> xv = *reinterpret_cast<const BVec<V>*>(input + a);
     BVec<V> zv;
@@ -425,7 +458,7 @@
       if (V == 1) bits = (__ballot_sync(group, bits) >> (lane & ~7u)) & 0xffu;
       if (V == 8 || lane % 8 == 0) mask[a >> 3] = (uint8_t)bits;
     }
-  }
+  });
 }
 
 struct PoolDims {
@@ -769,7 +802,7 @@
                                                              const bf16* __restrict__ input2, bf16* __restrict__ grad_input2,
                                                              const float* __restrict__ mean2, const float* __restrict__ inv_std2,
                                                              const float* __restrict__ weight2, const float* __restrict__ sum_dy_xmu2,
-                                                             const int reduction_size, const int stride) {
+                                                             const RowWalk walk, const int reduction_size, const int stride) {
   static_assert(!DUAL || (G == kGradY || G == kGradBits), "a dual tail derives g from dy and the ReLU");
   const float norm_fct = FCT_PTR ? *norm_fct_ptr : norm_fct_value;
   const int c0 = (blockIdx.x * blockDim.x + threadIdx.x) * V;
@@ -791,7 +824,7 @@
     }
   }
   const int row_step = blockDim.y * gridDim.y;
-  for (int m = blockIdx.y * blockDim.y + threadIdx.y; m < reduction_size; m += row_step) {
+  walk.visit(blockIdx.y * blockDim.y + threadIdx.y, row_step, reduction_size, [&](const int m) {
     const int a = m * stride + c0;
     const BVec<V> gv = *reinterpret_cast<const BVec<V>*>(grad_output + a);
     BVec<V> gv2, yv;
@@ -813,8 +846,8 @@
     }
     *reinterpret_cast<BVec<V>*>(grad_input + a) = dxv;
     if (DUAL) *reinterpret_cast<BVec<V>*>(grad_input2 + a) = dx2v;
-  }
-}
-
-}
-}
+  });
+}
+
+}
+}
diff --git a/ant-ray_b200/csrc/norm_launch.h b/ant-ray_b200/csrc/norm_launch.h
--- a/ant-ray_b200/csrc/norm_launch.h
+++ b/ant-ray_b200/csrc/norm_launch.h
@@ -70,6 +70,11 @@
 cudaError_t sync_bwd_elemt(const BwdArgs& a, cudaStream_t s);
 cudaError_t load_kernels();
 
+constexpr int kWalkFalling = 0;
+constexpr int kWalkGroups = 1;
+constexpr int kWalkRising = 2;
+int last_walk();
+
 struct InferParams {
   const void* weight;
   const void* bias;
diff --git a/include/b200coll.h b/include/b200coll.h
--- a/include/b200coll.h
+++ b/include/b200coll.h
@@ -176,6 +176,7 @@
 int b200c_debug_fill_flags(b200c_comm_t* comm, uint32_t value);
 
 size_t b200c_bn_scratch_bytes(int channels);
+int b200c_bn_last_walk(void);
 int b200c_bn_forward(const void* x, const void* identity, void* y, const float* weight, const float* bias,
                      float* running_mean, float* running_var, int64_t* num_batches_tracked, float* save_mean,
                      float* save_invstd, int m, int channels, float momentum, float eps, void* scratch,
```

Result: no change. 5707, median of 6 (+2.5%).
